# kabachuha/sd-webui-text2video

Hardware: NVIDIA H100
Metric: denoised frames/sec (UNet+VAE) ModelScope 24fx256^2 50-step (higher is better)
Workload: dtype f16 (fp32 accumulate / norms / softmax)

## Files before the change

### include/t2v_b200.h

```cpp
#ifndef T2V_B200_H
#define T2V_B200_H

#include <stddef.h>
#include <stdint.h>

#ifdef __cplusplus
extern "C" {
#endif

int t2v_init(int device);
const char* t2v_last_error(void);
int t2v_num_sms(void);
const char* t2v_version(void);

typedef struct t2v_unet t2v_unet;

typedef struct {
    int in_dim, dim, context_dim, out_dim;
    int dim_mult[8];
    int n_mult;
    int num_heads;
    int head_dim;
    int num_res_blocks;
    float attn_scales[8];
    int n_attn_scales;
    int arch;
    int temporal_length;
} t2v_unet_config;

int t2v_unet_create(const t2v_unet_config* cfg, t2v_unet** out);
void t2v_unet_destroy(t2v_unet* u);
int t2v_unet_set_param(t2v_unet* u, const char* name, const void* data, int dtype, int ndim, const int64_t* shape,
                       void* stream);
int t2v_unet_missing_params(t2v_unet* u, char* name_out, size_t name_cap);
int t2v_unet_param_info(t2v_unet* u, int index, char* name_out, size_t name_cap, int64_t* shape_out, int* ndim_out);
int t2v_unet_forward(t2v_unet* u, const void* x, int x_is_f32, const float* t, const void* ctx, void* out,
                     int out_is_f32, int B, int F, int h, int w, int L, void* stream);
int t2v_unet_forward_ctx(t2v_unet* u, const void* x, int x_is_f32, const float* t, const void* ctx, int ctx_B, void* out,
                         int out_is_f32, int B, int F, int h, int w, int L, void* stream);
int t2v_unet_forward_adapter(t2v_unet* u, const void* x, int x_is_f32, const float* t, const void* ctx,
                             const void* const* feats, int n_feats, int feats_B, void* out, int out_is_f32, int B, int F, int h,
                             int w, int L, void* stream);
double t2v_unet_flops(t2v_unet* u, int B, int F, int h, int w, int L);
int t2v_unet_plan_bytes(t2v_unet* u, int B, int F, int h, int w, int L, size_t* arena);
int t2v_unet_plan_info(t2v_unet* u, int B, int ctx_B, int F, int h, int w, int L, size_t* arena, double* flops, int* cached);
int t2v_unet_num_launches(t2v_unet* u);
int t2v_unet_profile(t2v_unet* u, int B, int F, int h, int w, int L, void* stream, double* out13);
long long t2v_unet_read_tap(t2v_unet* u, const char* name, void* dst, long long cap_elems, void* stream);
int t2v_unet_enable_taps(t2v_unet* u, int on);
int t2v_unet_tap_info(t2v_unet* u, const char* name, long long* rows, int* C, int* h, int* w);

int t2v_unet_lora_merge(t2v_unet* u, const char* weight_name, const void* lora_A, const void* lora_B, int rank, float alpha,
                        int temporal_mean, void* stream);
int t2v_unet_lora_clear(t2v_unet* u, void* stream);
int t2v_unet_lora_merged(t2v_unet* u);

int t2v_unet_lora_apply(t2v_unet* u, const char* weight_name, const void* up, const void* down, int dtype, int rank, float alpha,
                        void* stream);
int t2v_unet_lora_restore(t2v_unet* u, const char* weight_name, void* stream);

typedef struct {
    unsigned char comm_handle[64];
    unsigned char slab_handle[64];
    int rank, nranks;
    int n_exchanges, n_groupnorms;
    long long dst_offset[192];
} t2v_shard_export;
int t2v_unet_shard_setup(t2v_unet* u, int rank, int nranks);
int t2v_unet_shard_prepare(t2v_unet* u, int B, int F, int h, int w, int L, void* stream, t2v_shard_export* out);
int t2v_unet_shard_connect(t2v_unet* u, int B, int F, int h, int w, int L, const t2v_shard_export* all, void* stream);
int t2v_unet_shard_connected(t2v_unet* u, int B, int F, int h, int w, int L);
int t2v_unet_shard_barrier(t2v_unet* u, void* stream);
int t2v_unet_shard_info(t2v_unet* u, int F, int* frame_begin, int* frame_end, int* n_exchanges);

typedef struct t2v_vae t2v_vae;
typedef struct {
    int ch;
    int ch_mult[8];
    int n_mult;
    int num_res_blocks;
    int z_channels;
    int out_ch;
    int embed_dim;
} t2v_vae_config;
int t2v_vae_create(const t2v_vae_config* cfg, t2v_vae** out);
void t2v_vae_destroy(t2v_vae* v);
int t2v_vae_set_param(t2v_vae* v, const char* name, const void* data, int dtype, int ndim, const int64_t* shape,
                      void* stream);
int t2v_vae_missing_params(t2v_vae* v, char* name_out, size_t name_cap);
int t2v_vae_param_info(t2v_vae* v, int index, char* name_out, size_t name_cap, int64_t* shape_out, int* ndim_out);
int t2v_vae_decode(t2v_vae* v, const void* z, int z_is_f32, float z_scale, void* out, int out_mode, int B, int F, int h,
                   int w, void* stream);
int t2v_vae_encode(t2v_vae* v, const void* x, int x_is_f32, void* moments_out, int N, int H, int W, void* stream);
double t2v_vae_flops(t2v_vae* v, int nframes, int h, int w);
int t2v_vae_plan_bytes(t2v_vae* v, int direction, int frames, int h, int w, size_t* arena, size_t* gn_workspace);
int t2v_vae_plan_chunks(t2v_vae* v, int direction, int frames, int h, int w, size_t budget, int* chunk_frames, int* n_chunks);
int t2v_vae_set_memory_budget(t2v_vae* v, size_t bytes);
size_t t2v_vae_get_memory_budget(t2v_vae* v);
int t2v_vae_last_chunking(t2v_vae* v, int direction, int* chunk_frames, int* n_chunks);
int t2v_vae_cached_plans(t2v_vae* v, int direction, size_t* slab_bytes);
int t2v_vae_lora_apply(t2v_vae* v, const char* weight_name, const void* up, const void* down, int dtype, int rank, float alpha,
                       void* stream);
int t2v_vae_lora_restore(t2v_vae* v, const char* weight_name, void* stream);
int t2v_vae_lora_clear(t2v_vae* v, void* stream);
int t2v_vae_lora_merged(t2v_vae* v);

typedef struct t2v_clip t2v_clip;
typedef struct {
    int width;
    int heads;
    int layers_run;
    int context;
    int vocab;
    int arch;
} t2v_clip_config;
int t2v_clip_create(const t2v_clip_config* cfg, t2v_clip** out);
void t2v_clip_destroy(t2v_clip* m);
int t2v_clip_set_param(t2v_clip* m, const char* name, const void* data, int dtype, int ndim, const int64_t* shape, void* stream);
int t2v_clip_param_info(t2v_clip* m, int index, char* name_out, size_t name_cap, int64_t* shape_out, int* ndim_out);
int t2v_clip_encode(t2v_clip* m, const int* tokens, void* out, int out_is_f32, int B, void* stream);
int t2v_clip_lora_apply(t2v_clip* m, const char* weight_name, const void* up, const void* down, int dtype, int rank, float alpha,
                        void* stream);
int t2v_clip_lora_restore(t2v_clip* m, const char* weight_name, void* stream);
int t2v_clip_lora_clear(t2v_clip* m, void* stream);
int t2v_clip_lora_merged(t2v_clip* m);

typedef struct t2v_adapter t2v_adapter;
typedef struct {
    int cin;
    int channels[4];
    int n_levels;
    int nums_rb;
    int ksize;
    int sk;
    int use_conv;
} t2v_adapter_config;
int t2v_adapter_create(const t2v_adapter_config* cfg, t2v_adapter** out);
void t2v_adapter_destroy(t2v_adapter* a);
int t2v_adapter_set_param(t2v_adapter* a, const char* name, const void* data, int dtype, int ndim, const int64_t* shape,
                          void* stream);
int t2v_adapter_missing_params(t2v_adapter* a, char* name_out, size_t name_cap);
int t2v_adapter_param_info(t2v_adapter* a, int index, char* name_out, size_t name_cap, int64_t* shape_out, int* ndim_out);
int t2v_adapter_encode(t2v_adapter* a, const void* cond, int cond_is_f32, void* const* feats_out, int N, int H, int W,
                       void* stream);
int t2v_adapter_lora_apply(t2v_adapter* a, const char* weight_name, const void* up, const void* down, int dtype, int rank,
                           float alpha, void* stream);
int t2v_adapter_lora_restore(t2v_adapter* a, const char* weight_name, void* stream);
int t2v_adapter_lora_clear(t2v_adapter* a, void* stream);
int t2v_adapter_lora_merged(t2v_adapter* a);

int t2v_ddim_step(const float* x, const void* eps_c, const void* eps_u, int eps_is_f32, float* x_out, long long n,
                  long long chan_stride,
                  int C, int guided_channels, float g, int mode, float a0, float a1, float a2, float a3, float a4,
                  const float* noise, int cfg_fp16, void* stream);
int t2v_cfg_x0(const float* x, const void* eps_c, const void* eps_u, int eps_is_f32, float* x0, long long n, float g,
               float alpha, float sigma, int cfg_fp16, void* stream);
int t2v_lincomb(float* out, const float* const* src, const float* coef, int n_src, long long n, void* stream);

int t2v_latent_blend(const float* image_latents, int image_frames, const double* noise, const double* weights, double* out,
                     double* mask_out, int BC, int F, long long hw, void* stream);

int t2v_q_sample_blend(const float* x0, const long long* x0_strides, const float* noise, const long long* noise_strides,
                       const float* a, const float* s, const float* mask, const long long* mask_strides, const float* img,
                       float* out, const int* shape, void* stream);

int t2v_frames_resize(const void* src, int n, int H0, int W0, void* out, int H, int W, int out_fp16, void* tmp,
                      long long tmp_bytes, void* stream);
int t2v_resize_coeffs(int in_size, int out_size, int* ksize, int* bounds, int* coeffs);

int t2v_op_gemm(const void* a, long long lda, int K, int nd, const int* dims, int ntaps, const int* tap_off,
                const void* w_packed, int n_alloc, int N, int b_batch_dim, int flags, void* out, long long ldo,
                const void* bias, int bias_rows, long long bias_stride, const void* residual, long long ldr,
                float alpha, int force_bn, int force_cg, void* stream);
int t2v_op_gemm_splitk(const void* a, long long lda, int K, int nd, const int* dims, int ntaps, const int* tap_off,
                       const void* w_packed, int n_alloc, int N, int b_batch_dim, int flags, void* out, long long ldo,
                       const void* bias, int bias_rows, long long bias_stride, const void* residual, long long ldr,
                       float alpha, int splits, float* scratch, long long scratch_elems, int* splits_used, int force_bn,
                       int force_cg, void* stream);
int t2v_op_ln_linear(const void* x, long long ldx, long long rows, int K, const void* w, const void* bias, const void* gamma,
                     const void* beta, int N, int flags, void* w_folded, float* colsum, float* bias32, float* rowstat,
                     const void* residual, long long ldr, void* out, long long ldo, int force_bn, int force_cg, void* stream);
int t2v_op_pack_conv_weight(const void* src, int src_is_f32, void* dst, int Cout, int Cin, int taps, int n_alloc,
                            int k_alloc, void* stream);
int t2v_op_pack_geglu_weight(const void* w, const void* b, int src_is_f32, void* wdst, void* bdst, int H, int K, int bn,
                             void* stream);
int t2v_op_groupnorm(const void* x, long long ldx, void* y, long long ldy, long long rows, int C, int rows_per_inst,
                     const void* gamma, const void* beta, float eps, int silu, int phase, float* stats, void* stream);
int t2v_op_layernorm(const void* x, long long ldx, void* y, long long ldy, long long rows, int C, const void* gamma,
                     const void* beta, float eps, void* stream);
int t2v_op_attention(const void* q, const void* k, const void* v, void* o, long long q_bs, long long q_ss,
                     long long k_bs, long long k_ss, long long v_bs, long long v_ss, long long o_bs, long long o_ss,
                     int batch, int heads, int sq, int skv, int kv_batch_div, float scale, void* stream);
int t2v_op_attention_hd(const void* q, const void* k, const void* v, void* o, long long q_bs, long long q_ss,
                        long long k_bs, long long k_ss, long long v_bs, long long v_ss, long long o_bs, long long o_ss,
                        int batch, int heads, int head_dim, int sq, int skv, int kv_batch_div, float scale, int b_inner,
                        long long q_bsi, long long k_bsi, long long v_bsi, long long o_bsi, void* stream);
int t2v_op_attention_relpos(const void* q, const void* k, const void* v, void* o, const void* table_k, const void* table_v,
                            long long n_seq, long long seq_inner, long long bs_outer, long long bs_inner, long long ss,
                            long long o_bs_outer, long long o_bs_inner, long long o_ss, int heads, int head_dim, int T,
                            int max_rel, float scale, void* stream);
int t2v_op_clip_attention(const void* qkv, void* o, int B, int L, int W, int heads, void* stream);
int t2v_op_upsample2x(const void* x, void* y, int nframes, int h, int w, int C, void* stream);
int t2v_op_im2col_s2(const void* x, void* col, int nframes, int h, int w, int C, void* stream);
int t2v_op_time_sinusoid(const float* t, void* out, int B, int dim, void* stream);
int t2v_op_small_linear(const void* x, long long ldx, const void* W, const void* bias, const void* addend, void* y,
                        long long ldy, int B, int N, int K, int silu_in, void* stream);

#ifdef __cplusplus
}
#endif
#endif
```

### sd-webui-text2video_b200/csrc/api.cu

```cuda
#include "../../include/t2v_b200.h"
#include "common.cuh"
#include "gemm_tc.cuh"
#include "kernels.cuh"

#include <cstdarg>
#include <cstdio>
#include <cstring>

namespace t2v {

static char g_err[512] = "";
static int g_device = -1;
static int g_num_sms = 132;
static void* g_gn_ws = nullptr;
static size_t g_gn_ws_bytes = 0;

void set_error(const char* fmt, ...) {
    va_list ap;
    va_start(ap, fmt);
    vsnprintf(g_err, sizeof(g_err), fmt, ap);
    va_end(ap);
}
int num_sms() { return g_num_sms; }
void clear_pending_error(const char* where) {
    const cudaError_t e = cudaGetLastError();
    if (e != cudaSuccess)
        fprintf(stderr, "[t2v_b200] %s: clearing a pending CUDA error left by an earlier call: %s (%s)\n", where, cudaGetErrorString(e),
                cudaGetErrorName(e));
}
int launch_status(const char* what) {
    const cudaError_t e = cudaGetLastError();
    if (e == cudaSuccess) return 0;
    set_error("%s: %s (%s)", what, cudaGetErrorString(e), cudaGetErrorName(e));
    return -2;
}

static void* gn_scratch(size_t bytes) {
    if (bytes > g_gn_ws_bytes) {
        if (g_gn_ws) cudaFree(g_gn_ws);
        g_gn_ws = nullptr;
        if (cudaMalloc(&g_gn_ws, bytes) != cudaSuccess) return nullptr;
        cudaMemset(g_gn_ws, 0, bytes);
        g_gn_ws_bytes = bytes;
    }
    return g_gn_ws;
}

}

using namespace t2v;

extern "C" {

int t2v_init(int device) {
    if (cudaSetDevice(device) != cudaSuccess) {
        set_error("cudaSetDevice(%d) failed: %s", device, cudaGetErrorString(cudaGetLastError()));
        return -1;
    }
    cudaDeviceProp prop;
    if (cudaGetDeviceProperties(&prop, device) != cudaSuccess) {
        set_error("cudaGetDeviceProperties failed");
        return -1;
    }
    if (prop.major != 9 || prop.minor != 0) {
        set_error("t2v_b200 is built for sm_90a only; device %d is sm_%d%d", device, prop.major, prop.minor);
        return -2;
    }
    g_device = device;
    g_num_sms = prop.multiProcessorCount;
    if (gemm_init() != 0) {
        set_error("gemm_init failed (driver entry point / smem attribute)");
        return -3;
    }
    return 0;
}
const char* t2v_last_error(void) { return g_err; }
int t2v_num_sms(void) { return g_num_sms; }
const char* t2v_version(void) { return "t2v_b200 0.2 (sm_90a; wgmma+TMA implicit GEMM)"; }

}

static GemmProblem op_problem(const void* a, long long lda, int K, int nd, const int* dims, int ntaps, const int* tap_off,
                              const void* w_packed, int n_alloc, int N, int b_batch_dim, int flags, void* out, long long ldo,
                              const void* bias, int bias_rows, long long bias_stride, const void* residual, long long ldr,
                              float alpha, int force_bn, int force_cg) {
    GemmProblem p;
    memset(&p, 0, sizeof(p));
    p.a = reinterpret_cast<const __half*>(a);
    p.lda = lda;
    p.K = K;
    p.nd = nd;
    for (int d = 0; d < nd; ++d) p.dim[d] = dims[d];
    p.ntaps = ntaps;
    for (int t = 0; t < ntaps; ++t)
        for (int d = 0; d < nd; ++d) p.tap_off[t][d] = tap_off ? tap_off[t * nd + d] : 0;
    p.b = reinterpret_cast<const __half*>(w_packed);
    p.n_alloc = n_alloc;
    p.N = N;
    p.b_batch_dim = b_batch_dim;
    p.flags = flags & ~(GEMM_DBG_FORCE_BS | GEMM_DBG_NO_BS | GEMM_DBG_SLAB_OUT);
    p.force_bs = (flags & GEMM_DBG_FORCE_BS) ? 1 : ((flags & GEMM_DBG_NO_BS) ? -1 : 0);
    p.slab_out = (flags & GEMM_DBG_SLAB_OUT) ? 1 : 0;
    p.out = out;
    p.ldo = ldo;
    p.bias = reinterpret_cast<const __half*>(bias);
    p.bias_rows = bias_rows;
    p.bias_stride = bias_stride;
    p.residual = reinterpret_cast<const __half*>(residual);
    p.ldr = ldr;
    p.alpha = alpha;
    p.force_bn = force_bn;
    p.force_cg = force_cg;
    return p;
}

static int plan_op(const GemmProblem& p, GemmPlan* plan, const char* what) {
    const int rc = gemm_plan(p, plan, g_num_sms);
    if (rc != 0) set_error("%s: gemm_plan failed (%d)", what, rc);
    return rc;
}

static int launch_op(const GemmPlan& plan, const char* what, cudaStream_t stream) {
    const int rc = gemm_launch(plan, stream);
    if (rc != 0) set_error("%s: gemm_launch failed: %s", what, cudaGetErrorString(cudaGetLastError()));
    return rc;
}

extern "C" {

int t2v_op_gemm(const void* a, long long lda, int K, int nd, const int* dims, int ntaps, const int* tap_off,
                const void* w_packed, int n_alloc, int N, int b_batch_dim, int flags, void* out, long long ldo,
                const void* bias, int bias_rows, long long bias_stride, const void* residual, long long ldr,
                float alpha, int force_bn, int force_cg, void* stream) {
    const GemmProblem p = op_problem(a, lda, K, nd, dims, ntaps, tap_off, w_packed, n_alloc, N, b_batch_dim, flags, out, ldo, bias,
                                     bias_rows, bias_stride, residual, ldr, alpha, force_bn, force_cg);
    GemmPlan plan;
    const int rc = plan_op(p, &plan, "op_gemm");
    return rc != 0 ? rc : launch_op(plan, "op_gemm", reinterpret_cast<cudaStream_t>(stream));
}

int t2v_op_gemm_splitk(const void* a, long long lda, int K, int nd, const int* dims, int ntaps, const int* tap_off,
                       const void* w_packed, int n_alloc, int N, int b_batch_dim, int flags, void* out, long long ldo,
                       const void* bias, int bias_rows, long long bias_stride, const void* residual, long long ldr,
                       float alpha, int splits, float* scratch, long long scratch_elems, int* splits_used, int force_bn,
                       int force_cg, void* stream) {
    const GemmProblem p = op_problem(a, lda, K, nd, dims, ntaps, tap_off, w_packed, n_alloc, N, b_batch_dim, flags, out, ldo, bias,
                                     bias_rows, bias_stride, residual, ldr, alpha, force_bn, force_cg);
    if (const char* why = gemm_splitk_unsupported(p)) {
        set_error("op_gemm_splitk: split-K does not take this problem: %s", why);
        return -1;
    }
    if (splits < 1 || scratch == nullptr || splits_used == nullptr) {
        set_error("op_gemm_splitk: needs splits >= 1, a scratch buffer and a place for the split count");
        return -1;
    }
    const int S = gemm_split_count(p, splits);
    const long long need = gemm_splitk_scratch_elems(p, S);
    if (scratch_elems < need) {
        set_error("op_gemm_splitk: %d splits need %lld fp32 scratch elements, the buffer holds %lld", S, need, scratch_elems);
        return -1;
    }
    GemmPlan plan;
    int rc = plan_op(gemm_splitk_partials(p, S, scratch), &plan, "op_gemm_splitk");
    if (rc != 0) return rc;
    *splits_used = S;
    const cudaStream_t s = reinterpret_cast<cudaStream_t>(stream);
    rc = launch_op(plan, "op_gemm_splitk", s);
    if (rc != 0) return rc;
    rc = gemm_splitk_reduce(p, S, scratch, s);
    if (rc != 0) set_error("op_gemm_splitk: splitk_reduce failed (%d)", rc);
    return rc;
}

int t2v_op_ln_linear(const void* x, long long ldx, long long rows, int K, const void* w, const void* bias, const void* gamma,
                     const void* beta, int N, int flags, void* w_folded, float* colsum, float* bias32, float* rowstat,
                     const void* residual, long long ldr, void* out, long long ldo, int force_bn, int force_cg, void* stream) {
    if (!x || !w || !gamma || !beta || !w_folded || !colsum || !bias32 || !rowstat || !out) {
        set_error("op_ln_linear: x, w, gamma, beta, out and the four intermediate buffers are required");
        return -1;
    }
    if ((flags & ~GEMM_GEGLU) != 0) {
        set_error("op_ln_linear: flags must be 0 or GEMM_GEGLU (%d)", flags);
        return -1;
    }
    if (K % 8 != 0 || K > 2048 || rows < 1 || rows >= (1LL << 31) || N < 1) {
        set_error("op_ln_linear: LayerNorm rows need K %% 8 == 0 and K <= 2048, 1 <= rows < 2^31 (K %d rows %lld N %d)", K, rows, N);
        return -1;
    }
    GemmProblem p;
    memset(&p, 0, sizeof(p));
    p.a = reinterpret_cast<const __half*>(x);
    p.lda = ldx;
    p.K = K;
    p.nd = 1;
    p.dim[0] = static_cast<int>(rows);
    p.ntaps = 1;
    p.b = reinterpret_cast<const __half*>(w_folded);
    p.n_alloc = N;
    p.N = N;
    p.b_batch_dim = -1;
    p.flags = flags | GEMM_LN;
    p.out = out;
    p.ldo = ldo;
    p.residual = reinterpret_cast<const __half*>(residual);
    p.ldr = ldr;
    p.alpha = 1.0f;
    p.force_bn = force_bn;
    p.force_cg = force_cg;
    p.rowstat = reinterpret_cast<const float2*>(rowstat);
    p.colsum = colsum;
    p.bias32 = bias32;
    GemmPlan plan;
    int rc = plan_op(p, &plan, "op_ln_linear");
    if (rc != 0) return rc;
    const cudaStream_t s = reinterpret_cast<cudaStream_t>(stream);
    rc = fold_ln_into_linear(reinterpret_cast<const __half*>(w), reinterpret_cast<const __half*>(bias),
                             reinterpret_cast<const __half*>(gamma), reinterpret_cast<const __half*>(beta),
                             reinterpret_cast<__half*>(w_folded), colsum, bias32, N, K, s);
    if (rc == 0) rc = layernorm_rowstats(p.a, ldx, rows, K, 1e-5f, reinterpret_cast<float2*>(rowstat), s);
    if (rc != 0) {
        set_error("op_ln_linear: fold / row statistics launch failed (%d)", rc);
        return rc;
    }
    return launch_op(plan, "op_ln_linear", s);
}

int t2v_latent_blend(const float* image_latents, int image_frames, const double* noise, const double* weights, double* out,
                     double* mask_out, int BC, int F, long long hw, void* stream) {
    if ((image_frames != 1 && image_frames != F) || BC < 1 || F < 1 || hw < 1) {
        set_error("latent_blend: image_frames must be 1 or F");
        return -1;
    }
    return latent_blend(image_latents, image_frames, noise, weights, out, mask_out, BC, F, hw, reinterpret_cast<cudaStream_t>(stream));
}

int t2v_q_sample_blend(const float* x0, const long long* x0_strides, const float* noise, const long long* noise_strides,
                       const float* a, const float* s, const float* mask, const long long* mask_strides, const float* img,
                       float* out, const int* shape, void* stream) {
    if (!x0 || !x0_strides || !noise || !noise_strides || !a || !s || !out || !shape) {
        set_error("q_sample_blend: x0, noise, a, s, out, their strides and the shape are required");
        return -1;
    }
    if ((mask == nullptr) != (img == nullptr) || (mask && !mask_strides)) {
        set_error("q_sample_blend: mask and img go together (both null for q_sample), and a mask needs strides");
        return -1;
    }
    QSampleBlendParams p;
    memset(&p, 0, sizeof(p));
    p.x0 = x0;
    p.noise = noise;
    p.a = a;
    p.s = s;
    p.mask = mask;
    p.img = img;
    p.out = out;
    for (int d = 0; d < 5; ++d) {
        if (shape[d] < 1) {
            set_error("q_sample_blend: shape[%d] = %d, every dimension must be >= 1", d, shape[d]);
            return -1;
        }
        if (x0_strides[d] < 0 || noise_strides[d] < 0 || (mask && mask_strides[d] < 0)) {
            set_error("q_sample_blend: negative stride in dimension %d", d);
            return -1;
        }
        p.shape[d] = shape[d];
        p.x0_stride[d] = x0_strides[d];
        p.noise_stride[d] = noise_strides[d];
        p.mask_stride[d] = mask ? mask_strides[d] : 0;
    }
    return q_sample_blend(p, reinterpret_cast<cudaStream_t>(stream));
}

int t2v_resize_coeffs(int in_size, int out_size, int* ksize, int* bounds, int* coeffs) {
    if (ksize == nullptr || resize_table(in_size, out_size, ksize, bounds, coeffs) != 0) {
        set_error("resize_coeffs: sizes must lie in [1, %d] (in %d, out %d) and ksize must not be null", kResizeMaxSize, in_size,
                  out_size);
        return -1;
    }
    return 0;
}

int t2v_frames_resize(const void* src, int n, int H0, int W0, void* out, int H, int W, int out_fp16, void* tmp,
                      long long tmp_bytes, void* stream) {
    const int M = kResizeMaxSize;
    if (n < 1 || H0 < 1 || W0 < 1 || H < 1 || W < 1 || H0 > M || W0 > M || H > M || W > M) {
        set_error("frames_resize: n must be >= 1 and every size in [1, %d] (n %d, %dx%d -> %dx%d)", M, n, W0, H0, W, H);
        return -1;
    }
    if (src == nullptr || out == nullptr) {
        set_error("frames_resize: src and out are required");
        return -1;
    }
    const size_t esize = out_fp16 ? sizeof(__half) : sizeof(float);
    if (reinterpret_cast<uintptr_t>(out) % esize != 0) {
        set_error("frames_resize: out must be aligned to its element size (%zu bytes)", esize);
        return -1;
    }
    const long long need = W != W0 ? static_cast<long long>(n) * H0 * W * 3 : 0;
    if (W != W0 && (tmp == nullptr || tmp_bytes < need)) {
        set_error("frames_resize: resizing %d to %d columns needs a uint8 buffer of %lld bytes, got %lld", W0, W, need,
                  tmp ? tmp_bytes : 0LL);
        return -1;
    }
    clear_pending_error("frames_resize");
    return frames_resize(static_cast<const uint8_t*>(src), n, H0, W0, out, H, W, out_fp16, static_cast<uint8_t*>(tmp),
                         reinterpret_cast<cudaStream_t>(stream));
}

int t2v_op_pack_conv_weight(const void* src, int src_is_f32, void* dst, int Cout, int Cin, int taps, int n_alloc,
                            int k_alloc, void* stream) {
    return pack_conv_weight(src, src_is_f32, reinterpret_cast<__half*>(dst), Cout, Cin, taps, n_alloc, k_alloc,
                            reinterpret_cast<cudaStream_t>(stream));
}
int t2v_op_pack_geglu_weight(const void* w, const void* b, int src_is_f32, void* wdst, void* bdst, int H, int K, int bn,
                             void* stream) {
    return pack_geglu_weight(w, b, src_is_f32, reinterpret_cast<__half*>(wdst), reinterpret_cast<__half*>(bdst), H, K, bn,
                             reinterpret_cast<cudaStream_t>(stream));
}
int t2v_op_groupnorm(const void* x, long long ldx, void* y, long long ldy, long long rows, int C, int rows_per_inst,
                     const void* gamma, const void* beta, float eps, int silu, int phase, float* stats, void* stream) {
    const __half* xh = reinterpret_cast<const __half*>(x);
    __half* yh = reinterpret_cast<__half*>(y);
    const __half* gh = reinterpret_cast<const __half*>(gamma);
    const __half* bh = reinterpret_cast<const __half*>(beta);
    if (phase < 0 || phase > 2 || (phase != 0 && stats == nullptr)) {
        set_error("op_groupnorm: phase %d must be 0, 1 or 2, and phases 1 and 2 need a stats buffer", phase);
        return -1;
    }
    if (groupnorm_check(xh, ldx, yh, ldy, rows, C, rows_per_inst, gh, bh) != 0) return -1;
    const int n_inst = static_cast<int>(rows / rows_per_inst);
    void* ws = gn_scratch(gn_workspace_bytes(rows_per_inst, n_inst, g_num_sms));
    if (!ws) {
        set_error("groupnorm workspace allocation failed");
        return -5;
    }
    const cudaStream_t s = reinterpret_cast<cudaStream_t>(stream);
    const size_t stats_bytes = static_cast<size_t>(n_inst) * 32 * sizeof(float2);
    if (phase == 2 && cudaMemcpyAsync(gn_workspace_stats(ws), stats, stats_bytes, cudaMemcpyDeviceToDevice, s) != cudaSuccess)
        return launch_status("op_groupnorm: statistics copy");
    const int rc = groupnorm_silu(xh, ldx, yh, ldy, rows, C, rows_per_inst, gh, bh, eps, silu, ws, g_num_sms, s, phase);
    if (rc != 0 || phase != 1) return rc;
    if (cudaMemcpyAsync(stats, gn_workspace_stats(ws), stats_bytes, cudaMemcpyDeviceToDevice, s) != cudaSuccess)
        return launch_status("op_groupnorm: statistics copy");
    return 0;
}
int t2v_op_layernorm(const void* x, long long ldx, void* y, long long ldy, long long rows, int C, const void* gamma,
                     const void* beta, float eps, void* stream) {
    return layernorm(reinterpret_cast<const __half*>(x), ldx, reinterpret_cast<__half*>(y), ldy, rows, C,
                     reinterpret_cast<const __half*>(gamma), reinterpret_cast<const __half*>(beta), eps,
                     reinterpret_cast<cudaStream_t>(stream));
}
int t2v_op_attention(const void* q, const void* k, const void* v, void* o, long long q_bs, long long q_ss,
                     long long k_bs, long long k_ss, long long v_bs, long long v_ss, long long o_bs, long long o_ss,
                     int batch, int heads, int sq, int skv, int kv_batch_div, float scale, void* stream) {
    AttnParams p;
    p.q = reinterpret_cast<const __half*>(q);
    p.k = reinterpret_cast<const __half*>(k);
    p.v = reinterpret_cast<const __half*>(v);
    p.o = reinterpret_cast<__half*>(o);
    p.q_bs = q_bs; p.q_ss = q_ss; p.k_bs = k_bs; p.k_ss = k_ss; p.v_bs = v_bs; p.v_ss = v_ss; p.o_bs = o_bs; p.o_ss = o_ss;
    p.batch = batch; p.heads = heads; p.sq = sq; p.skv = skv; p.head_dim = 64; p.kv_batch_div = kv_batch_div;
    p.scale = scale; p.b_inner = 1; p.q_bsi = p.k_bsi = p.v_bsi = p.o_bsi = 0;
    return attention(p, reinterpret_cast<cudaStream_t>(stream));
}
int t2v_op_attention_hd(const void* q, const void* k, const void* v, void* o, long long q_bs, long long q_ss,
                        long long k_bs, long long k_ss, long long v_bs, long long v_ss, long long o_bs, long long o_ss,
                        int batch, int heads, int head_dim, int sq, int skv, int kv_batch_div, float scale, int b_inner,
                        long long q_bsi, long long k_bsi, long long v_bsi, long long o_bsi, void* stream) {
    AttnParams p;
    memset(&p, 0, sizeof(p));
    p.q = reinterpret_cast<const __half*>(q);
    p.k = reinterpret_cast<const __half*>(k);
    p.v = reinterpret_cast<const __half*>(v);
    p.o = reinterpret_cast<__half*>(o);
    p.q_bs = q_bs; p.q_ss = q_ss; p.k_bs = k_bs; p.k_ss = k_ss; p.v_bs = v_bs; p.v_ss = v_ss; p.o_bs = o_bs; p.o_ss = o_ss;
    p.batch = batch; p.heads = heads; p.sq = sq; p.skv = skv; p.head_dim = head_dim; p.kv_batch_div = kv_batch_div;
    p.scale = scale; p.b_inner = b_inner;
    p.q_bsi = q_bsi; p.k_bsi = k_bsi; p.v_bsi = v_bsi; p.o_bsi = o_bsi;
    return attention(p, reinterpret_cast<cudaStream_t>(stream));
}
int t2v_op_attention_relpos(const void* q, const void* k, const void* v, void* o, const void* table_k, const void* table_v,
                            long long n_seq, long long seq_inner, long long bs_outer, long long bs_inner, long long ss,
                            long long o_bs_outer, long long o_bs_inner, long long o_ss, int heads, int head_dim, int T,
                            int max_rel, float scale, void* stream) {
    RelposParams p;
    memset(&p, 0, sizeof(p));
    p.q = reinterpret_cast<const __half*>(q);
    p.k = reinterpret_cast<const __half*>(k);
    p.v = reinterpret_cast<const __half*>(v);
    p.o = reinterpret_cast<__half*>(o);
    p.table_k = reinterpret_cast<const __half*>(table_k);
    p.table_v = reinterpret_cast<const __half*>(table_v);
    p.n_seq = n_seq; p.seq_inner = seq_inner; p.bs_outer = bs_outer; p.bs_inner = bs_inner; p.ss = ss;
    p.o_bs_outer = o_bs_outer; p.o_bs_inner = o_bs_inner; p.o_ss = o_ss;
    p.heads = heads; p.head_dim = head_dim; p.T = T; p.max_rel = max_rel; p.scale = scale;
    return attention_relpos(p, reinterpret_cast<cudaStream_t>(stream));
}
int t2v_op_upsample2x(const void* x, void* y, int nframes, int h, int w, int C, void* stream) {
    return upsample2x(reinterpret_cast<const __half*>(x), reinterpret_cast<__half*>(y), nframes, h, w, C,
                      reinterpret_cast<cudaStream_t>(stream));
}
int t2v_op_im2col_s2(const void* x, void* col, int nframes, int h, int w, int C, void* stream) {
    return im2col_s2(reinterpret_cast<const __half*>(x), reinterpret_cast<__half*>(col), nframes, h, w, C,
                     reinterpret_cast<cudaStream_t>(stream));
}
int t2v_op_time_sinusoid(const float* t, void* out, int B, int dim, void* stream) {
    return time_sinusoid(t, reinterpret_cast<__half*>(out), B, dim, reinterpret_cast<cudaStream_t>(stream));
}
int t2v_op_small_linear(const void* x, long long ldx, const void* W, const void* bias, const void* addend, void* y,
                        long long ldy, int B, int N, int K, int silu_in, void* stream) {
    return small_linear(reinterpret_cast<const __half*>(x), ldx, reinterpret_cast<const __half*>(W),
                        reinterpret_cast<const __half*>(bias), reinterpret_cast<const __half*>(addend),
                        reinterpret_cast<__half*>(y), ldy, B, N, K, silu_in, reinterpret_cast<cudaStream_t>(stream));
}
int t2v_ddim_step(const float* x, const void* eps_c, const void* eps_u, int eps_is_f32, float* x_out, long long n, long long chan_stride,
                  int C, int guided_channels, float g, int mode, float a0, float a1, float a2, float a3, float a4,
                  const float* noise, int cfg_fp16, void* stream) {
    DdimStepParams p;
    p.x = x; p.eps_c = eps_c; p.eps_u = eps_u; p.eps_is_f32 = eps_is_f32;
    p.x_out = x_out; p.n = n; p.chan_stride = chan_stride; p.C = C; p.guided_channels = guided_channels; p.g = g;
    p.mode = mode; p.a0 = a0; p.a1 = a1; p.a2 = a2; p.a3 = a3; p.a4 = a4; p.noise = noise; p.cfg_fp16 = cfg_fp16;
    return ddim_step(p, reinterpret_cast<cudaStream_t>(stream));
}
int t2v_cfg_x0(const float* x, const void* eps_c, const void* eps_u, int eps_is_f32, float* x0, long long n, float g, float alpha,
               float sigma, int cfg_fp16, void* stream) {
    return cfg_x0(x, eps_c, eps_u, eps_is_f32, x0, n, g, alpha, sigma,
                  cfg_fp16, reinterpret_cast<cudaStream_t>(stream));
}
int t2v_lincomb(float* out, const float* const* src, const float* coef, int n_src, long long n, void* stream) {
    return lincomb(out, src, coef, n_src, n, reinterpret_cast<cudaStream_t>(stream));
}

}
```

### sd-webui-text2video_b200/csrc/gemm_tc.cu

```cuda
#include "common.cuh"
#include "gemm_tc.cuh"
#include "kernels.cuh"
#include "ptx.cuh"

#include <algorithm>
#include <cstdio>
#include <cstdlib>
#include <cstring>

namespace t2v {

namespace {

constexpr int kThreads = 384;
constexpr int kRegsProducer = 40;
constexpr int kRegsConsumer = 232;
constexpr int kABytes = GEMM_BLOCK_M * GEMM_BLOCK_K * 2;
constexpr int kSmemPerBlock = 227 * 1024;
constexpr int kSmemBudget = 216 * 1024;
constexpr int kMaxStages = 8;
constexpr int kEpiRowBytes = 128;
constexpr int kSlabBytes = 8 * 8 * kEpiRowBytes;
constexpr int kRowTabBytes = 8 * 16 * 4;

__host__ __device__ constexpr int out_chunk_cols(int outw) { return outw >= 32 ? 32 : 16; }
__host__ __device__ constexpr int out_chunks(int outw) { return (outw + out_chunk_cols(outw) - 1) / out_chunk_cols(outw); }

template <int BN, bool SLAB = false>
struct Cfg {
    static constexpr int kBBytes = BN * GEMM_BLOCK_K * 2;
    static constexpr int kStageBytes = kABytes + kBBytes;
    static constexpr int kColBytes = BN * 8;
    static constexpr int kTailBytes = 1024  + 256  + kRowTabBytes + kColBytes;
    static constexpr int kOutBytes = SLAB ? kSlabBytes : std::max(kSlabBytes, out_chunks(BN) * GEMM_BLOCK_M * out_chunk_cols(BN) * 2);
    static constexpr int kStages = std::min(kMaxStages, (kSmemPerBlock - kTailBytes - kOutBytes) / kStageBytes);
    static constexpr int kSmemBytes = kStages * kStageBytes + kOutBytes + kTailBytes;
    static constexpr int kBsSmemBytes = kSmemBudget + kSlabBytes + kTailBytes;
    static_assert(kSmemBytes <= kSmemPerBlock, "shared memory per block");
};
static_assert(Cfg<256>::kStages == 3 && Cfg<224>::kStages == 3 && Cfg<192>::kStages == 4 && Cfg<160>::kStages == 5 &&
                  Cfg<128>::kStages == 6 && Cfg<64>::kStages == 8 && Cfg<16>::kStages == 8,
              "ring depths next to the output tile");
static_assert(Cfg<256, true>::kStages == 4 && Cfg<224, true>::kStages == 4, "ring depths without the output tile");

__device__ __forceinline__ float gelu_erf(float x) {
    const float z = fabsf(x) * 0.70710678118654752440f;
    float t;
    asm("rcp.approx.ftz.f32 %0, %1;" : "=f"(t) : "f"(fmaf(0.3275911f, z, 1.0f)));
    float p = fmaf(t, 0.5f * 1.061405429f, 0.5f * -1.453152027f);
    p = fmaf(p, t, 0.5f * 1.421413741f);
    p = fmaf(p, t, 0.5f * -0.284496736f);
    p = fmaf(p, t, 0.5f * 0.254829592f);
    const float q = p * t * ex2_approx(z * z * -1.4426950408889634f);
    return x * (x < 0.f ? q : 1.0f - q);
}

__device__ __forceinline__ uint32_t stg_off(int r, int b, int segs) {
    const int L = r * segs + (b >> 4);
    return static_cast<uint32_t>(((L ^ ((L >> 3) & 7)) << 4) | (b & 15));
}

template <int BN, bool GEGLU>
__device__ __forceinline__ void epilogue_affine(const GemmDesc& g, float (&acc)[BN / 2], const uint8_t* cols, const int* rowg,
                                                const float2 (&rs)[2], int tn, int lane) {
    const int quad = lane & 3, fr = lane >> 2;
    if (!GEGLU && g.bias != nullptr && g.bias_rows > 0 && (g.flags & GEMM_LN) == 0) {
        const int col0 = tn * BN + 2 * quad;
        const int nrem = g.N - col0;
        const __half* brow[2];
#pragma unroll
        for (int h = 0; h < 2; ++h) {
            const int fg = rowg[fr + 8 * h];
            brow[h] = g.bias + (fg >= 0 ? (fg / g.bias_rows) * g.bias_stride : 0) + col0;
        }
#pragma unroll
        for (int j = 0; j < BN / 8; ++j) {
#pragma unroll
            for (int e = 0; e < 2; ++e) {
                if (8 * j + e >= nrem) continue;
                acc[4 * j + e] = fmaf(acc[4 * j + e], g.alpha, __half2float(__ldg(brow[0] + 8 * j + e)));
                acc[4 * j + 2 + e] = fmaf(acc[4 * j + 2 + e], g.alpha, __half2float(__ldg(brow[1] + 8 * j + e)));
            }
        }
        return;
    }
    const bool ln = (g.flags & GEMM_LN) != 0;
#pragma unroll
    for (int j = 0; j < BN / 8; ++j) {
        const int c = 8 * j + 2 * quad;
        if (ln) {
            const float4 p = *reinterpret_cast<const float4*>(cols + 8 * c);
            acc[4 * j] = fmaf(rs[0].y, fmaf(-rs[0].x, p.x, acc[4 * j]), p.y);
            acc[4 * j + 2] = fmaf(rs[1].y, fmaf(-rs[1].x, p.x, acc[4 * j + 2]), p.y);
            acc[4 * j + 1] = fmaf(rs[0].y, fmaf(-rs[0].x, p.z, acc[4 * j + 1]), p.w);
            acc[4 * j + 3] = fmaf(rs[1].y, fmaf(-rs[1].x, p.z, acc[4 * j + 3]), p.w);
        } else {
            const float2 b = __half22float2(*reinterpret_cast<const __half2*>(cols + 2 * c));
            acc[4 * j] = fmaf(acc[4 * j], g.alpha, b.x);
            acc[4 * j + 2] = fmaf(acc[4 * j + 2], g.alpha, b.x);
            acc[4 * j + 1] = fmaf(acc[4 * j + 1], g.alpha, b.y);
            acc[4 * j + 3] = fmaf(acc[4 * j + 3], g.alpha, b.y);
        }
    }
}

template <int BN>
struct ResQ {
    static constexpr int kCW = kEpiRowBytes / 2;
    static constexpr int kUnits = 2 * ((BN + kCW - 1) / kCW);
    static constexpr int kDepth = BN <= 192 ? kUnits : 4;
    static __device__ __forceinline__ int segs(int c) { return (min(kCW, BN - c * kCW) * 2) / 16; }
    static __device__ __forceinline__ void load(const GemmDesc& g, const int* rowg, int tn, int u, int lane, uint4 (&rb)[2]) {
        const int c = u >> 1, h = u & 1, sg = segs(c);
        const bool vec_res = (g.ldr & 7) == 0 && (reinterpret_cast<uintptr_t>(g.residual) & 15) == 0;
#pragma unroll
        for (int p = 0; p < 2; ++p) {
            const int idx = lane + 32 * p;
            rb[p] = make_uint4(0u, 0u, 0u, 0u);
            if (idx >= 8 * sg) continue;
            const int gr = rowg[8 * h + idx / sg];
            const int col = tn * BN + c * kCW + 8 * (idx % sg);
            if (gr < 0) continue;
            const __half* src = g.residual + gr * g.ldr + col;
            if (vec_res && col + 8 <= g.N) {
                rb[p] = __ldg(reinterpret_cast<const uint4*>(src));
            } else {
                uint32_t w[4];
#pragma unroll
                for (int e = 0; e < 4; ++e) {
                    const __half2 v = __halves2half2(col + 2 * e < g.N ? src[2 * e] : __ushort_as_half(0),
                                                     col + 2 * e + 1 < g.N ? src[2 * e + 1] : __ushort_as_half(0));
                    w[e] = *reinterpret_cast<const uint32_t*>(&v);
                }
                rb[p] = make_uint4(w[0], w[1], w[2], w[3]);
            }
        }
    }
};

template <int BN, bool GEGLU, bool F32>
__device__ __forceinline__ void epilogue_warp(const GemmDesc& g, float (&acc)[BN / 2], uint4 (&rq)[ResQ<BN>::kDepth][2],
                                              uint8_t* stg, const int* rowg, int tn, int sp, int lane) {
    static_assert(!(GEGLU && F32), "GEGLU stores fp16");
    constexpr bool RES = !GEGLU && !F32;
    constexpr int ES = F32 ? 4 : 2;
    constexpr int EPS = 16 / ES;
    constexpr int OUTW = GEGLU ? BN / 2 : BN;
    constexpr int CW = kEpiRowBytes / ES;
    constexpr int NCH = (OUTW + CW - 1) / CW;
    constexpr int NU = 2 * NCH;
    constexpr int QD = ResQ<BN>::kDepth;
    const int quad = lane & 3, fr = lane >> 2;
    const int nvalid = GEGLU ? g.N / 2 : g.N;
    const int ocol0 = tn * OUTW;
    const bool has_res = RES && g.residual != nullptr;
    const bool vec_out = (g.ldo % EPS) == 0 && (reinterpret_cast<uintptr_t>(g.out) & 15) == 0 && (!F32 || (g.split_stride % EPS) == 0);

    auto segs_of = [](int c) { return (min(CW, OUTW - c * CW) * ES) / 16; };
#pragma unroll
    for (int u = 0; u < NU; ++u) {
        const int c = u >> 1, h = u & 1, segs = segs_of(c);
        if (RES && has_res) {
#pragma unroll
            for (int p = 0; p < 2; ++p) {
                const int idx = lane + 32 * p;
                if (idx < 8 * segs) *reinterpret_cast<uint4*>(stg + stg_off(idx / segs, 16 * (idx % segs), segs)) = rq[u % QD][p];
            }
            if (u + QD < NU) ResQ<BN>::load(g, rowg, tn, u + QD, lane, rq[u % QD]);
            __syncwarp();
        }
#pragma unroll
        for (int jj = 0; jj < CW / 8; ++jj) {
            if (jj >= segs * EPS / 8) break;
            const int j = c * (CW / 8) + jj;
            uint8_t* sp_ = stg + stg_off(fr, (8 * jj + 2 * quad) * ES, segs);
            float v0 = acc[4 * j + 2 * h], v1 = acc[4 * j + 2 * h + 1];
            if constexpr (GEGLU) {
                const __half2 xh = __floats2half2_rn(v0, v1);
                const float2 gf = __half22float2(__floats2half2_rn(acc[BN / 4 + 4 * j + 2 * h], acc[BN / 4 + 4 * j + 2 * h + 1]));
                const __half2 ge = __floats2half2_rn(gelu_erf(gf.x), gelu_erf(gf.y));
                *reinterpret_cast<__half2*>(sp_) = __hmul2(xh, ge);
            } else if constexpr (F32) {
                *reinterpret_cast<float2*>(sp_) = make_float2(v0, v1);
            } else {
                if (has_res) {
                    const float2 f = __half22float2(*reinterpret_cast<const __half2*>(sp_));
                    v0 += f.x;
                    v1 += f.y;
                }
                *reinterpret_cast<__half2*>(sp_) = __floats2half2_rn(v0, v1);
            }
        }
        __syncwarp();
#pragma unroll
        for (int p = 0; p < 2; ++p) {
            const int idx = lane + 32 * p;
            if (idx >= 8 * segs) continue;
            const int gr = rowg[8 * h + idx / segs];
            if (gr < 0) continue;
            const int col = ocol0 + c * CW + EPS * (idx % segs);
            const uint4 val = *reinterpret_cast<const uint4*>(stg + stg_off(idx / segs, 16 * (idx % segs), segs));
            uint8_t* dst = static_cast<uint8_t*>(g.out) + ((F32 ? sp * g.split_stride : 0) + gr * g.ldo + col) * ES;
            if (vec_out && col + EPS <= nvalid) {
                *reinterpret_cast<uint4*>(dst) = val;
            } else {
                const uint32_t w[4] = {val.x, val.y, val.z, val.w};
#pragma unroll
                for (int e = 0; e < EPS; ++e)
                    if (col + e < nvalid) {
                        if constexpr (F32) reinterpret_cast<uint32_t*>(dst)[e] = w[e];
                        else reinterpret_cast<uint16_t*>(dst)[e] = static_cast<uint16_t>(w[e >> 1] >> (16 * (e & 1)));
                    }
            }
        }
        __syncwarp();
    }
}

__device__ __forceinline__ void tile_origin(const GemmDesc& g, int tmi, int (&org)[GEMM_MAX_RDIMS]) {
#pragma unroll
    for (int d = 0; d < GEMM_MAX_RDIMS; ++d) org[d] = 0;
    if (g.nd == 1) {
        org[0] = tmi * g.box[0];
        return;
    }
    int tm = tmi;
#pragma unroll
    for (int d = 0; d < GEMM_MAX_RDIMS; ++d) {
        if (d < g.nd) {
            const int td = g.tdim[d];
            const int qd = tm / td;
            org[d] = (tm - qd * td) * g.box[d];
            tm = qd;
        }
    }
}

__device__ __forceinline__ void tma_store_box(const CUtensorMap* map, const void* src, int nd, int c0, const int (&org)[GEMM_MAX_RDIMS]) {
    if (nd == 1) tma_store_2d(map, src, c0, org[0]);
    else if (nd == 2) tma_store_3d(map, src, c0, org[0], org[1]);
    else if (nd == 3) tma_store_4d(map, src, c0, org[0], org[1], org[2]);
    else tma_store_5d(map, src, c0, org[0], org[1], org[2], org[3]);
}
__device__ __forceinline__ void tma_load_box(void* dst, const CUtensorMap* map, uint64_t* bar, int nd, int c0,
                                             const int (&org)[GEMM_MAX_RDIMS]) {
    if (nd == 1) tma_load_2d(dst, map, bar, c0, org[0]);
    else if (nd == 2) tma_load_3d(dst, map, bar, c0, org[0], org[1]);
    else if (nd == 3) tma_load_4d(dst, map, bar, c0, org[0], org[1], org[2]);
    else tma_load_5d(dst, map, bar, c0, org[0], org[1], org[2], org[3]);
}

template <int OCW>
__device__ __forceinline__ int out_unit_swizzle(int r) { return ((r * OCW * 2) >> 7) & (OCW / 8 - 1); }

template <int BN, bool GEGLU>
__device__ __forceinline__ int live_out_chunks(const GemmDesc& g, int tn) {
    constexpr int OUTW = GEGLU ? BN / 2 : BN;
    constexpr int OCW = out_chunk_cols(OUTW);
    return min(out_chunks(OUTW), ((GEGLU ? g.N / 2 : g.N) - tn * OUTW + OCW - 1) / OCW);
}

template <int BN, bool GEGLU>
__device__ __forceinline__ void epilogue_tile(const GemmDesc& g, const float (&acc)[BN / 2], uint8_t* tile, uint64_t* tilefree,
                                              uint32_t tphase, uint64_t* tilefull, int r0, int lane) {
    constexpr int OUTW = GEGLU ? BN / 2 : BN;
    constexpr int OCW = out_chunk_cols(OUTW);
    const int quad = lane & 3, fr = lane >> 2;
    const bool has_res = !GEGLU && g.residual != nullptr;
    const uint32_t row = smem_u32(tile) + static_cast<uint32_t>((r0 + fr) * (OCW * 2) + 4 * quad);
    const int sw = out_unit_swizzle<OCW>(r0 + fr);
    mbar_wait(tilefree, tphase);
#pragma unroll
    for (int j = 0; j < OUTW / 8; ++j) {
#pragma unroll
        for (int h = 0; h < 2; ++h) {
            const uint32_t p = row + (j / (OCW / 8)) * (GEMM_BLOCK_M * OCW * 2) + 8 * h * (OCW * 2) + (((j % (OCW / 8)) ^ sw) << 4);
            float v0 = acc[4 * j + 2 * h], v1 = acc[4 * j + 2 * h + 1];
            __half2 v;
            if constexpr (GEGLU) {
                const __half2 xh = __floats2half2_rn(v0, v1);
                const float2 gf = __half22float2(__floats2half2_rn(acc[BN / 4 + 4 * j + 2 * h], acc[BN / 4 + 4 * j + 2 * h + 1]));
                v = __hmul2(xh, __floats2half2_rn(gelu_erf(gf.x), gelu_erf(gf.y)));
            } else {
                if (has_res) {
                    const uint32_t rw = ld_shared_u32(p);
                    const float2 f = __half22float2(*reinterpret_cast<const __half2*>(&rw));
                    v0 += f.x;
                    v1 += f.y;
                }
                v = __floats2half2_rn(v0, v1);
            }
            st_shared_u32(p, *reinterpret_cast<const uint32_t*>(&v));
        }
    }
    fence_proxy_async_smem();
    __syncwarp();
    if (lane == 0) mbar_arrive(tilefull);
}

template <int BN, bool GEGLU, int CG, bool BS = false, bool SLAB = false>
__global__ void __launch_bounds__(kThreads, 1) gemm_tc_kernel(const __grid_constant__ GemmDesc g) {
    using Cf = Cfg<BN, SLAB>;
    static_assert(!BS || CG == 1, "B-stationary tiles are single-CTA");
    static_assert(!BS || Cf::kBsSmemBytes <= kSmemPerBlock, "shared memory per block");
    constexpr int kBarStages = BS ? kMaxStages : Cf::kStages;
    const uint32_t rank = CG == 2 ? cluster_ctarank() : 0u;
    extern __shared__ uint8_t smem_raw[];
    const uint32_t raw = smem_u32(smem_raw);
    uint8_t* smem = smem_raw + (((raw + 1023u) & ~1023u) - raw);
    uint8_t* const epi = smem + (BS ? kSmemBudget : Cf::kStages * Cf::kStageBytes);
    uint64_t* bars = reinterpret_cast<uint64_t*>(epi + (BS ? kSlabBytes : Cf::kOutBytes));
    uint64_t* full = bars;
    uint64_t* empty = bars + kBarStages;
    uint64_t* bfull = empty + kBarStages;
    uint64_t* colfull = bfull + 1;
    uint64_t* colempty = bfull + 2;
    uint64_t* tilefree = bfull + 3;
    uint64_t* tilefull = bfull + 4;
    int* const rowtab = reinterpret_cast<int*>(reinterpret_cast<uint8_t*>(bars) + 256);
    uint8_t* const cols = reinterpret_cast<uint8_t*>(rowtab) + kRowTabBytes;
    const bool tma_out = !BS && !SLAB && g.tma_out != 0;
    const int nst = BS ? g.bs_stages : Cf::kStages;
    uint8_t* const sB_res = smem;
    uint8_t* const sA_ring = smem + (BS ? g.ntaps * g.k_chunks * Cf::kBBytes : 0);

    const int wg = threadIdx.x >> 7;

    if (threadIdx.x == 0) {
        tma_prefetch_desc(&g.map_a);
        tma_prefetch_desc(&g.map_b);
        if (tma_out) {
            tma_prefetch_desc(&g.map_o);
            if (g.residual != nullptr) tma_prefetch_desc(&g.map_r);
        }
        for (int i = 0; i < kBarStages; ++i) {
            mbar_init(&full[i], 1);
            mbar_init(&empty[i], 2 * CG);
        }
        if constexpr (BS) mbar_init(bfull, 1);
        mbar_init(colfull, 1);
        mbar_init(colempty, 8);
        mbar_init(tilefree, 1);
        mbar_init(tilefull, 8);
        fence_barrier_init();
    }
    if constexpr (CG == 2) cluster_sync_all();
    else __syncthreads();

    const int pairs_m = (g.tiles_m + CG - 1) / CG;
    const int nsplit = g.splits > 1 ? g.splits : 1;
    const int total_pairs = pairs_m * g.tiles_n * nsplit;
    const int k_total = g.ntaps * g.k_chunks;
    const int k_per = g.splits > 1 ? g.k_per_split : k_total;
    const int bs_tn = BS ? static_cast<int>(blockIdx.x) % g.tiles_n : 0;
    const int first_pair = BS ? static_cast<int>(blockIdx.x) / g.tiles_n : static_cast<int>(blockIdx.x) / CG;
    const int pair_stride = BS ? (static_cast<int>(gridDim.x) - bs_tn + g.tiles_n - 1) / g.tiles_n : static_cast<int>(gridDim.x) / CG;
    const int total_items = BS ? g.tiles_m : total_pairs;
    const bool col_operands = (g.flags & GEMM_LN) != 0 || g.bias == nullptr || g.bias_rows == 0;

    if (wg == 0) {
        setmaxnreg_dec<kRegsProducer>();
        if (threadIdx.x < 32 && elect_one()) {
            int stage = 0;
            uint32_t phase = 0;
            if constexpr (BS) {
                if (first_pair < total_items) {
                    mbar_expect_tx(bfull, static_cast<uint32_t>(k_total * Cf::kBBytes));
                    const int kch0 = g.k_chunks;
                    for (int it = 0, tap = 0, kc = 0; it < k_total; ++it) {
                        tma_load_3d(sB_res + it * Cf::kBBytes, &g.map_b, bfull, kc * GEMM_BLOCK_K, bs_tn * BN, tap);
                        if (++kc == kch0) {
                            kc = 0;
                            ++tap;
                        }
                    }
                }
            }
            const int kch = g.k_chunks, nd = g.nd, a_tx = g.a_tx_bytes, tiles_n_ = g.tiles_n, tiles_m_ = g.tiles_m;
            const int bdim = g.b_batch_dim;
            for (int wi = first_pair; wi < total_items; wi += pair_stride) {
                int sp = 0, pt = wi;
                if (!BS && nsplit > 1) {
                    sp = wi % nsplit;
                    pt = wi / nsplit;
                }
                const int it0 = sp * k_per, it1 = min(k_total, it0 + k_per);
                int tn = bs_tn, tmi = wi;
                if constexpr (!BS) {
                    const int pm = pt / tiles_n_;
                    tn = pt - pm * tiles_n_;
                    tmi = pm * CG + static_cast<int>(rank);
                }
                int org[GEMM_MAX_RDIMS];
                tile_origin(g, tmi, org);
                if (tmi >= tiles_m_) org[0] = g.dim[0];
                const int bbatch = bdim < 0 ? 0 : (bdim == 0 ? org[0] : (bdim == 1 ? org[1] : (bdim == 2 ? org[2] : org[3])));
                int tap = 0, kc = it0;
                if (it0 >= kch) {
                    tap = it0 / kch;
                    kc = it0 - tap * kch;
                }
                int c1 = org[0] + g.tap_off[tap][0], c2 = org[1] + g.tap_off[tap][1];
                int c3 = org[2] + g.tap_off[tap][2], c4 = org[3] + g.tap_off[tap][3];
                for (int it = it0; it < it1; ++it) {
                    mbar_wait(&empty[stage], phase ^ 1u);
                    uint8_t* sa = BS ? sA_ring + stage * kABytes : smem + stage * Cf::kStageBytes;
                    uint8_t* sb = sa + kABytes;
                    const int k0 = kc * GEMM_BLOCK_K;
                    mbar_expect_tx(&full[stage], static_cast<uint32_t>(a_tx + (BS ? 0 : Cf::kBBytes)));
                    if (nd == 1) tma_load_2d(sa, &g.map_a, &full[stage], k0, c1);
                    else if (nd == 2) tma_load_3d(sa, &g.map_a, &full[stage], k0, c1, c2);
                    else if (nd == 3) tma_load_4d(sa, &g.map_a, &full[stage], k0, c1, c2, c3);
                    else tma_load_5d(sa, &g.map_a, &full[stage], k0, c1, c2, c3, c4);
                    if constexpr (CG == 2) {
                        constexpr int kHalf = BN / 2;
                        tma_load_3d_mc(sb + rank * (kHalf * GEMM_BLOCK_K * 2), &g.map_b, &full[stage], k0,
                                       tn * BN + static_cast<int>(rank) * kHalf, tap + bbatch, static_cast<uint16_t>(3));
                    } else if constexpr (!BS) {
                        tma_load_3d(sb, &g.map_b, &full[stage], k0, tn * BN, tap + bbatch);
                    }
                    if (++kc == kch) {
                        kc = 0;
                        ++tap;
                        if (it + 1 < it1) {
                            c1 = org[0] + g.tap_off[tap][0];
                            c2 = org[1] + g.tap_off[tap][1];
                            c3 = org[2] + g.tap_off[tap][2];
                            c4 = org[3] + g.tap_off[tap][3];
                        }
                    }
                    if (++stage == nst) {
                        stage = 0;
                        phase ^= 1u;
                    }
                }
            }
        } else if (threadIdx.x >= 32 && threadIdx.x < 64 && col_operands) {
            const int lane = threadIdx.x & 31;
            const bool ln = (g.flags & GEMM_LN) != 0;
            uint32_t cphase = 0;
            for (int wi = first_pair; wi < total_items; wi += pair_stride) {
                const int col0 = (BS ? bs_tn : (wi / nsplit) % g.tiles_n) * BN;
                mbar_wait(colempty, cphase ^ 1u);
#pragma unroll
                for (int c = lane; c < BN; c += 32) {
                    const int col = col0 + c;
                    if (ln) {
                        reinterpret_cast<float2*>(cols)[c] =
                            col < g.N ? make_float2(__ldg(g.colsum + col), __ldg(g.bias32 + col)) : make_float2(0.f, 0.f);
                    } else {
                        reinterpret_cast<__half*>(cols)[c] = g.bias != nullptr && col < g.N ? __ldg(g.bias + col) : __ushort_as_half(0);
                    }
                }
                __syncwarp();
                if (lane == 0) mbar_arrive(colfull);
                cphase ^= 1u;
            }
        } else if (threadIdx.x >= 64 && threadIdx.x < 96 && tma_out) {
            if (elect_one()) {
                constexpr int OUTW = GEGLU ? BN / 2 : BN;
                constexpr int OCW = out_chunk_cols(OUTW);
                constexpr int kChunkBytes = GEMM_BLOCK_M * OCW * 2;
                const bool has_res = !GEGLU && g.residual != nullptr;
                const uint32_t box_bytes = static_cast<uint32_t>(g.a_tx_bytes / GEMM_BLOCK_K * OCW);
                uint32_t fphase = 0;
                for (int wi = first_pair; wi < total_items; wi += pair_stride) {
                    const int pt = wi / nsplit;
                    const int tn = pt % g.tiles_n;
                    const int tmi = (pt / g.tiles_n) * CG + static_cast<int>(rank);
                    const int nch = tmi < g.tiles_m ? live_out_chunks<BN, GEGLU>(g, tn) : 0;
                    int org[GEMM_MAX_RDIMS];
                    tile_origin(g, tmi, org);
                    if (has_res && nch > 0) {
                        mbar_expect_tx(tilefree, nch * box_bytes);
                        for (int c = 0; c < nch; ++c)
                            tma_load_box(epi + c * kChunkBytes, &g.map_r, tilefree, g.nd, tn * OUTW + c * OCW, org);
                    } else {
                        mbar_arrive(tilefree);
                    }
                    mbar_wait(tilefull, fphase);
                    fphase ^= 1u;
                    for (int c = 0; c < nch; ++c) tma_store_box(&g.map_o, epi + c * kChunkBytes, g.nd, tn * OUTW + c * OCW, org);
                    bulk_commit_group();
                    bulk_wait_group_read_0();
                }
                bulk_wait_group_0();
            }
        }
        __syncwarp();
    } else {
        setmaxnreg_inc<kRegsConsumer>();
        const int cw = wg - 1;
        const int lt = threadIdx.x & 127;
        const int wr = lt >> 5, lane = lt & 31;
        int stage = 0;
        uint32_t phase = 0;
        if constexpr (BS) {
            if (first_pair < total_items) mbar_wait(bfull, 0u);
        }
        const bool out_f32 = (g.flags & GEMM_OUT_F32) != 0;
        const bool ln = (g.flags & GEMM_LN) != 0;
        uint8_t* const stg = epi + (cw * 4 + wr) * (8 * kEpiRowBytes);
        int* const rowg = rowtab + (cw * 4 + wr) * 16;
        uint32_t cphase = 0, tphase = 0;
        float acc[BN / 2];
        uint4 rq[ResQ<BN>::kDepth][2];
        for (int wi = first_pair; wi < total_items; wi += pair_stride) {
            const int sp = BS ? 0 : wi % nsplit;
            const int pt = wi / nsplit;
            const int tn = BS ? bs_tn : pt % g.tiles_n;
            const int tmi = BS ? wi : (pt / g.tiles_n) * CG + static_cast<int>(rank);
            const int it0s = BS ? 0 : sp * k_per;
            const int k_iters = min(g.ntaps * g.k_chunks, it0s + k_per) - it0s;

            if (lane < 16) {
                const int r = cw * 64 + wr * 16 + lane;
                int grow = -1;
                if (tmi < g.tiles_m) {
                    if (g.nd == 1) {
                        const int o = tmi * g.box[0];
                        if (r < g.box[0] && o + r < g.dim[0]) grow = o + r;
                    } else {
                        int tm = tmi, rr = r;
                        long long mul = 1, gr = 0;
                        bool valid = true;
#pragma unroll
                        for (int d = 0; d < GEMM_MAX_RDIMS; ++d) {
                            const int td = g.tdim[d];
                            const int c = (tm % td) * g.box[d] + rr % g.box[d];
                            tm /= td;
                            rr /= g.box[d];
                            valid = valid && (c < g.dim[d]);
                            gr += mul * c;
                            mul *= g.dim[d];
                        }
                        if (valid && rr == 0) grow = static_cast<int>(gr);
                    }
                }
                rowg[lane] = grow;
            }
            __syncwarp();
            float2 rs[2];
#pragma unroll
            for (int h = 0; h < 2; ++h) {
                const int fg = rowg[(lane >> 2) + 8 * h];
                rs[h] = ln && fg >= 0 ? __ldg(g.rowstat + fg) : make_float2(0.f, 1.f);
            }

            int prev = -1;
#pragma unroll
            for (int i = 0; i < BN / 2; ++i) reg_fence(acc[i]);
            for (int it = 0; it < k_iters; ++it) {
                mbar_wait(&full[stage], phase);
                const uint32_t sa = smem_u32(BS ? sA_ring + stage * kABytes : smem + stage * Cf::kStageBytes) + cw * (64 * 128);
                const uint32_t sb = BS ? smem_u32(sB_res + it * Cf::kBBytes) : smem_u32(smem + stage * Cf::kStageBytes) + kABytes;
                const uint64_t da = wgmma_desc_sw128(sa);
                const uint64_t db = wgmma_desc_sw128(sb);
                wgmma_fence();
#pragma unroll
                for (int k = 0; k < GEMM_BLOCK_K / 16; ++k)
                    wgmma_ss<BN>(acc, da + static_cast<uint64_t>(k * 2), db + static_cast<uint64_t>(k * 2), (it | k) != 0 ? 1u : 0u);
                wgmma_commit();
                wgmma_wait<1>();
                if (prev >= 0 && lt == 0) {
                    mbar_arrive(&empty[prev]);
                    if constexpr (CG == 2) mbar_arrive_cluster(&empty[prev], rank ^ 1u);
                }
                prev = stage;
                if (++stage == nst) {
                    stage = 0;
                    phase ^= 1u;
                }
            }
            if constexpr (!GEGLU) {
                if (!tma_out && g.residual != nullptr) {
#pragma unroll
                    for (int u = 0; u < ResQ<BN>::kDepth; ++u) ResQ<BN>::load(g, rowg, tn, u, lane, rq[u]);
                }
            }
            wgmma_wait<0>();
#pragma unroll
            for (int i = 0; i < BN / 2; ++i) reg_fence(acc[i]);
            if (prev >= 0 && lt == 0) {
                mbar_arrive(&empty[prev]);
                if constexpr (CG == 2) mbar_arrive_cluster(&empty[prev], rank ^ 1u);
            }

            uint32_t ring = static_cast<uint32_t>(stage) | (phase << 16);
            asm volatile("" : "+r"(ring));
            if (col_operands) mbar_wait(colfull, cphase);
            epilogue_affine<BN, GEGLU>(g, acc, cols, rowg, rs, tn, lane);
            if (col_operands) {
                __syncwarp();
                if (lane == 0) mbar_arrive(colempty);
                cphase ^= 1u;
            }
            if (tma_out) {
                epilogue_tile<BN, GEGLU>(g, acc, epi, tilefree, tphase, tilefull, cw * 64 + wr * 16, lane);
                tphase ^= 1u;
            } else if constexpr (GEGLU) {
                epilogue_warp<BN, true, false>(g, acc, rq, stg, rowg, tn, sp, lane);
            } else if (out_f32) {
                epilogue_warp<BN, false, true>(g, acc, rq, stg, rowg, tn, sp, lane);
            } else {
                epilogue_warp<BN, false, false>(g, acc, rq, stg, rowg, tn, sp, lane);
            }
            asm volatile("" : "+r"(ring));
            stage = static_cast<int>(ring & 0xffffu);
            phase = ring >> 16;
        }
    }
    if constexpr (CG == 2) cluster_sync_all();
}

typedef CUresult (*EncodeTiledFn)(CUtensorMap*, CUtensorMapDataType, cuuint32_t, void*, const cuuint64_t*,
                                  const cuuint64_t*, const cuuint32_t*, const cuuint32_t*, CUtensorMapInterleave,
                                  CUtensorMapSwizzle, CUtensorMapL2promotion, CUtensorMapFloatOOBfill);
EncodeTiledFn g_encode = nullptr;
bool g_inited = false;

int encode_map(CUtensorMap* m, const void* base, int rank, const cuuint64_t* dims, const cuuint64_t* strides_bytes,
               const cuuint32_t* box, CUtensorMapSwizzle swizzle = CU_TENSOR_MAP_SWIZZLE_128B) {
    cuuint32_t estr[5] = {1, 1, 1, 1, 1};
    CUresult r = g_encode(m, CU_TENSOR_MAP_DATA_TYPE_FLOAT16, static_cast<cuuint32_t>(rank), const_cast<void*>(base),
                          dims, strides_bytes, box, estr, CU_TENSOR_MAP_INTERLEAVE_NONE, swizzle,
                          CU_TENSOR_MAP_L2_PROMOTION_L2_256B, CU_TENSOR_MAP_FLOAT_OOB_FILL_NONE);
    if (r != CUDA_SUCCESS) {
        fprintf(stderr, "[t2v] cuTensorMapEncodeTiled failed: %d (rank %d, dims %llu %llu %llu %llu %llu)\n",
                static_cast<int>(r), rank, (unsigned long long)dims[0], (unsigned long long)(rank > 1 ? dims[1] : 0),
                (unsigned long long)(rank > 2 ? dims[2] : 0), (unsigned long long)(rank > 3 ? dims[3] : 0),
                (unsigned long long)(rank > 4 ? dims[4] : 0));
        return -1;
    }
    return 0;
}

struct Variant {
    int bn, geglu, cg, smem;
    const void* fn;
    int bs, slab;
};
template <int BN, bool G, int CG>
Variant variant() {
    return Variant{BN, G ? 1 : 0, CG, Cfg<BN>::kSmemBytes, reinterpret_cast<const void*>(&gemm_tc_kernel<BN, G, CG>), 0, 0};
}
template <int BN, bool G>
Variant variant_bs() {
    return Variant{BN, G ? 1 : 0, 1, Cfg<BN>::kBsSmemBytes, reinterpret_cast<const void*>(&gemm_tc_kernel<BN, G, 1, true>), 1, 0};
}
template <int BN>
Variant variant_slab() {
    return Variant{BN, 0, 1, Cfg<BN, true>::kSmemBytes, reinterpret_cast<const void*>(&gemm_tc_kernel<BN, false, 1, false, true>), 0, 1};
}
const Variant* variants(int* n) {
    static const Variant v[] = {
        variant<16, false, 1>(),  variant<64, false, 1>(),  variant<128, false, 1>(), variant<160, false, 1>(),
        variant<192, false, 1>(), variant<224, false, 1>(),
        variant<256, false, 1>(), variant<64, true, 1>(),   variant<128, true, 1>(),  variant<256, true, 1>(),
        variant<64, false, 2>(),  variant<128, false, 2>(), variant<160, false, 2>(), variant<256, false, 2>(),
        variant<64, true, 2>(),   variant<128, true, 2>(),  variant<256, true, 2>(),
        variant_bs<160, false>(), variant_bs<128, false>(), variant_bs<128, true>(), variant_bs<64, false>(),
        variant_slab<224>(),      variant_slab<256>(),
    };
    *n = static_cast<int>(sizeof(v) / sizeof(v[0]));
    return v;
}
const Variant* find_variant(int bn, bool geglu, int cg, int bs, int slab) {
    int n;
    const Variant* v = variants(&n);
    for (int i = 0; i < n; ++i)
        if (v[i].bn == bn && v[i].geglu == (geglu ? 1 : 0) && v[i].cg == cg && v[i].bs == bs && v[i].slab == slab) return &v[i];
    return nullptr;
}

}

int gemm_init() {
    if (g_inited) return 0;
    void* fn = nullptr;
    cudaDriverEntryPointQueryResult qres;
    if (cudaGetDriverEntryPoint("cuTensorMapEncodeTiled", &fn, cudaEnableDefault, &qres) != cudaSuccess ||
        fn == nullptr) {
        fprintf(stderr, "[t2v] cuTensorMapEncodeTiled entry point not found\n");
        return -1;
    }
    g_encode = reinterpret_cast<EncodeTiledFn>(fn);
    int nv = 0;
    const Variant* vs = variants(&nv);
    bool attr_fail = false;
    for (int i = 0; i < nv; ++i)
        if (cudaFuncSetAttribute(vs[i].fn, cudaFuncAttributeMaxDynamicSharedMemorySize, vs[i].smem) != cudaSuccess) attr_fail = true;
    if (attr_fail) {
        fprintf(stderr, "[t2v] cudaFuncSetAttribute(max dynamic smem) failed: %s\n",
                cudaGetErrorString(cudaGetLastError()));
        return -1;
    }
    g_inited = true;
    return 0;
}

int tma_encode_f16(CUtensorMap* m, const void* base, int rank, const unsigned long long* dims,
                   const unsigned long long* strides_bytes, const unsigned* box) {
    if (gemm_init() != 0) return -1;
    cuuint64_t d[5], st[5];
    cuuint32_t bx[5];
    for (int i = 0; i < rank; ++i) {
        d[i] = dims[i];
        bx[i] = box[i];
        if (i + 1 < rank) st[i] = strides_bytes[i];
    }
    return encode_map(m, base, rank, d, st, bx);
}

static int gemm_bs_bn(long long tiles_m, int N, int K, int ntaps, int num_sms, int force_bn, bool any_k, int* stages_out) {
    static const bool bs_off = getenv("T2V_NO_BSTAT") != nullptr;
    static const int bs_kmax = getenv("T2V_BSTAT_KMAX") ? atoi(getenv("T2V_BSTAT_KMAX")) : 0;
    const int kt = ntaps * ((K + GEMM_BLOCK_K - 1) / GEMM_BLOCK_K);
    if (bs_off || N <= 16 || (kt > bs_kmax && !any_k)) return 0;
    const int cands[3] = {160, 128, 64};
    for (int i = 0; i < 3; ++i) {
        const int c = cands[i];
        if (force_bn != 0 && force_bn != c) continue;
        const int tn = (N + c - 1) / c;
        if (static_cast<double>(N) / (static_cast<double>(tn) * c) < 0.9) continue;
        const long long b_bytes = static_cast<long long>(kt) * c * GEMM_BLOCK_K * 2;
        if (b_bytes > kSmemBudget - 4 * kABytes || tn > num_sms) continue;
        const int stages = static_cast<int>(std::min<long long>(8, (kSmemBudget - b_bytes) / kABytes));
        const int group = num_sms / tn;
        if (tiles_m < 3LL * group) continue;
        if (stages_out) *stages_out = stages;
        return c;
    }
    return 0;
}

int gemm_plan(const GemmProblem& p, GemmPlan* plan, int num_sms) {
    if (gemm_init() != 0) return -1;
    if (p.nd < 1 || p.nd > GEMM_MAX_RDIMS || p.ntaps < 1 || p.ntaps > GEMM_MAX_TAPS) return -2;
    if ((p.lda & 7) != 0 || (p.K & 7) != 0 || (reinterpret_cast<uintptr_t>(p.a) & 15) != 0 ||
        (reinterpret_cast<uintptr_t>(p.b) & 15) != 0) {
        fprintf(stderr, "[t2v] gemm_plan: operands must be 16-byte aligned (lda %lld K %d)\n", p.lda, p.K);
        return -3;
    }
    GemmDesc& g = plan->desc;
    memset(&g, 0, sizeof(g));
    g.nd = p.nd;
    long long rows = 1;
    int remaining = GEMM_BLOCK_M;
    int boxrows = 1;
    for (int d = 0; d < GEMM_MAX_RDIMS; ++d) {
        const int ext = d < p.nd ? p.dim[d] : 1;
        g.dim[d] = ext;
        int b = std::min(ext, remaining);
        if (b < 1) b = 1;
        g.box[d] = b;
        g.tdim[d] = (ext + b - 1) / b;
        remaining = b >= ext ? remaining / b : 1;
        boxrows *= b;
        rows *= ext;
    }
    if (rows >= (1LL << 31)) {
        fprintf(stderr, "[t2v] gemm_plan: %lld rows, at most 2^31 - 1\n", rows);
        return -4;
    }
    if (p.b_batch_dim >= 0 && g.box[p.b_batch_dim] != 1) {
        const int d = p.b_batch_dim;
        boxrows /= g.box[d];
        g.box[d] = 1;
        g.tdim[d] = g.dim[d];
        for (int e = d + 1; e < GEMM_MAX_RDIMS; ++e) {
            boxrows /= g.box[e];
            g.box[e] = 1;
            g.tdim[e] = g.dim[e];
        }
    }
    g.tiles_m = 1;
    for (int d = 0; d < GEMM_MAX_RDIMS; ++d) g.tiles_m *= g.tdim[d];
    g.a_tx_bytes = boxrows * GEMM_BLOCK_K * 2;
    g.ntaps = p.ntaps;
    g.k_chunks = (p.K + GEMM_BLOCK_K - 1) / GEMM_BLOCK_K;
    for (int t = 0; t < p.ntaps; ++t)
        for (int d = 0; d < GEMM_MAX_RDIMS; ++d) g.tap_off[t][d] = static_cast<int8_t>(d < p.nd ? p.tap_off[t][d] : 0);
    g.b_batch_dim = p.b_batch_dim;
    g.N = p.N;
    g.flags = p.flags;
    g.out = p.out;
    g.ldo = p.ldo;
    g.bias = p.bias;
    g.bias_rows = p.bias_rows;
    g.bias_stride = p.bias_stride;
    g.residual = p.residual;
    g.ldr = p.ldr;
    g.alpha = p.alpha == 0.f ? 1.0f : p.alpha;
    g.rowstat = p.rowstat;
    g.colsum = p.colsum;
    g.bias32 = p.bias32;
    g.splits = gemm_split_count(p, p.splits);
    g.k_per_split = (g.ntaps * g.k_chunks + g.splits - 1) / g.splits;
    g.split_stride = p.split_stride;

    int bn = p.force_bn;
    const int k_total_sel = p.ntaps * g.k_chunks;
    if (bn == 0 && k_total_sel >= 10) {
        const int cands[7] = {256, 224, 192, 160, 128, 64, 16};
        double best = 1e30;
        for (int i = 0; i < 7; ++i) {
            const int c = cands[i];
            if ((p.flags & GEMM_GEGLU) && c != 256 && c != 128 && c != 64) continue;
            if (c == 16 && p.N > 16) continue;
            if (c > 16 && p.N <= 16) continue;
            if ((c == 224 || c == 192) && ((p.flags & GEMM_GEGLU) || p.b_batch_dim >= 0 || p.splits > 1)) continue;
            const int tn = (p.N + c - 1) / c;
            if ((p.flags & GEMM_GEGLU) && (p.N % c) != 0) continue;
            const long long tiles = static_cast<long long>(tn) * g.tiles_m * g.splits;
            const long long ctas = std::min<long long>(tiles, num_sms);
            const long long per_cta = (tiles + ctas - 1) / ctas;
            const int k_iters = g.splits > 1 ? (k_total_sel + g.splits - 1) / g.splits : k_total_sel;
            const double t_iter = std::max(650.0, 2.7 * c);
            const int chunks_per_warp = c >= 64 ? (c / 32 + 1) / 2 : 1;
            const double t_epi = 900.0 + chunks_per_warp * (p.residual != nullptr ? 2100.0 : 1050.0);
            const double t_tile = std::max(k_iters * t_iter, t_epi) + 1500.0;
            const double fit = static_cast<double>(p.N) / (static_cast<double>(tn) * c);
            const double t = (per_cta * t_tile + t_epi) * (1.0 + 0.02 * (1.0 - fit));
            if (t < best) {
                best = t;
                bn = c;
            }
        }
    }
    if (bn == 0) {
        const int cands[5] = {256, 160, 128, 64, 16};
        const double eff[5] = {1.0, 0.86, 0.80, 0.55, 0.25};
        double best = -1;
        for (int i = 0; i < 5; ++i) {
            const int c = cands[i];
            if ((p.flags & GEMM_GEGLU) && c != 256 && c != 128 && c != 64) continue;
            if (c == 16 && p.N > 16) continue;
            if (c > 16 && p.N <= 16) continue;
            const int tn = (p.N + c - 1) / c;
            const double waste = static_cast<double>(p.N) / (static_cast<double>(tn) * c);
            const long long tiles = static_cast<long long>(tn) * g.tiles_m;
            const long long waves = (tiles + num_sms - 1) / num_sms;
            const double fill = static_cast<double>(tiles) / (static_cast<double>(waves) * num_sms);
            const double score = eff[i] * waste * fill;
            if (score > best) {
                best = score;
                bn = c;
            }
        }
    }
    plan->bs = 0;
    if (!(p.flags & GEMM_GEGLU) && p.force_bs >= 0 && p.force_cg <= 1 && p.splits <= 1 && p.b_batch_dim < 0) {
        int stages = 0;
        const int c = gemm_bs_bn(g.tiles_m, p.N, p.K, p.ntaps, num_sms, p.force_bn, p.force_bs == 1, &stages);
        if (c > 0) {
            bn = c;
            plan->bs = 1;
            g.bs_stages = stages;
        }
    }
    plan->bn = bn;
    static const bool use_pairs = getenv("T2V_2CTA") != nullptr;
    plan->cg = p.force_cg ? p.force_cg : ((g.tiles_m >= 2 && bn >= 64 && use_pairs) ? 2 : 1);
    if (bn < 64 || p.b_batch_dim >= 0 || plan->bs || bn == 192 || bn == 224) plan->cg = 1;
    g.tiles_n = (p.N + bn - 1) / bn;
    if ((p.flags & GEMM_OUT_F32) && p.residual != nullptr) {
        fprintf(stderr, "[t2v] gemm_plan: fp32 output takes no residual\n");
        return -4;
    }
    if ((p.flags & GEMM_GEGLU) && (p.N % bn) != 0) {
        fprintf(stderr, "[t2v] gemm_plan: GEGLU needs N %% BN == 0 (N %d BN %d)\n", p.N, bn);
        return -4;
    }
    if ((p.flags & GEMM_GEGLU) && ((p.ldo & 15) != 0 || (reinterpret_cast<uintptr_t>(p.out) & 31) != 0 || p.residual != nullptr ||
                                   (p.flags & GEMM_OUT_F32) || p.bias_rows != 0 || p.splits > 1)) {
        fprintf(stderr, "[t2v] gemm_plan: GEGLU epilogue needs 32-byte aligned fp16 output rows (ldo %lld), no residual, "
                        "no per-sample bias, no split-K\n", p.ldo);
        return -4;
    }

    {
        cuuint64_t dims[5], strides[4];
        cuuint32_t box[5];
        dims[0] = static_cast<cuuint64_t>(p.K);
        box[0] = GEMM_BLOCK_K;
        long long pitch = p.lda * 2;
        for (int d = 0; d < p.nd; ++d) {
            dims[d + 1] = static_cast<cuuint64_t>(g.dim[d]);
            box[d + 1] = static_cast<cuuint32_t>(g.box[d]);
            strides[d] = static_cast<cuuint64_t>(pitch);
            pitch *= g.dim[d];
        }
        if (encode_map(&g.map_a, p.a, p.nd + 1, dims, strides, box) != 0) return -5;
    }
    {
        const int nb = p.b_batch_dim >= 0 ? g.dim[p.b_batch_dim] : p.ntaps;
        cuuint64_t dims[3] = {static_cast<cuuint64_t>(p.K), static_cast<cuuint64_t>(p.n_alloc),
                              static_cast<cuuint64_t>(nb)};
        const cuuint64_t ldb = static_cast<cuuint64_t>(p.ldb > 0 ? p.ldb : p.K);
        cuuint64_t strides[2] = {ldb * 2, ldb * 2 * static_cast<cuuint64_t>(p.n_alloc)};
        cuuint32_t box[3] = {GEMM_BLOCK_K, static_cast<cuuint32_t>(bn / plan->cg), 1};
        if (encode_map(&g.map_b, p.b, 3, dims, strides, box) != 0) return -6;
    }
    const auto tma_rows = [](const void* ptr, long long ld) { return (reinterpret_cast<uintptr_t>(ptr) & 15) == 0 && (ld & 7) == 0; };
    g.tma_out = !(p.flags & GEMM_OUT_F32) && !plan->bs && !p.slab_out && tma_rows(p.out, p.ldo) &&
                (p.residual == nullptr || tma_rows(p.residual, p.ldr));
    const long long tiles_all = static_cast<long long>(g.tiles_m) * g.tiles_n * g.splits;
    plan->slab = !plan->bs && plan->cg == 1 && !(p.flags & GEMM_GEGLU) && (bn == 224 || bn == 256) &&
                 (!g.tma_out || tiles_all <= num_sms) ? 1 : 0;
    if (plan->slab) g.tma_out = 0;
    if (g.tma_out) {
        const int outw = (p.flags & GEMM_GEGLU) ? bn / 2 : bn;
        const int ocw = out_chunk_cols(outw);
        cuuint64_t dims[5];
        cuuint64_t strides[4];
        cuuint32_t box[5];
        dims[0] = static_cast<cuuint64_t>((p.flags & GEMM_GEGLU) ? p.N / 2 : p.N);
        box[0] = static_cast<cuuint32_t>(ocw);
        for (int d = 0; d < p.nd; ++d) {
            dims[d + 1] = static_cast<cuuint64_t>(g.dim[d]);
            box[d + 1] = static_cast<cuuint32_t>(g.box[d]);
        }
        const CUtensorMapSwizzle sw = ocw == 32 ? CU_TENSOR_MAP_SWIZZLE_64B : CU_TENSOR_MAP_SWIZZLE_32B;
        for (int which = 0; which < (p.residual != nullptr ? 2 : 1); ++which) {
            long long pitch = (which == 0 ? p.ldo : p.ldr) * 2;
            for (int d = 0; d < p.nd; ++d) {
                strides[d] = static_cast<cuuint64_t>(pitch);
                pitch *= g.dim[d];
            }
            if (encode_map(which == 0 ? &g.map_o : &g.map_r, which == 0 ? p.out : p.residual, p.nd + 1, dims, strides, box, sw) != 0)
                return -8;
        }
    }
    const Variant* var = find_variant(bn, (p.flags & GEMM_GEGLU) != 0, plan->cg, plan->bs, plan->slab);
    if (var == nullptr) return -7;
    const long long pairs = static_cast<long long>((g.tiles_m + plan->cg - 1) / plan->cg) * g.tiles_n * g.splits;
    plan->grid = plan->cg * static_cast<int>(std::min<long long>(pairs, num_sms / plan->cg));
    if (plan->bs) plan->grid = (num_sms / g.tiles_n) * g.tiles_n;
    plan->smem = var->smem;
    plan->flops = 2.0 * static_cast<double>(rows) * p.N * p.K * p.ntaps;
    return 0;
}

int gemm_launch(const GemmPlan& plan, cudaStream_t stream) {
    const Variant* var = find_variant(plan.bn, (plan.desc.flags & GEMM_GEGLU) != 0, plan.cg, plan.bs, plan.slab);
    if (var == nullptr) return -1;
    cudaLaunchConfig_t cfg;
    memset(&cfg, 0, sizeof(cfg));
    cfg.gridDim = dim3(static_cast<unsigned>(plan.grid));
    cfg.blockDim = dim3(static_cast<unsigned>(kThreads));
    cfg.dynamicSmemBytes = static_cast<size_t>(plan.smem);
    cfg.stream = stream;
    cudaLaunchAttribute attr;
    attr.id = cudaLaunchAttributeClusterDimension;
    attr.val.clusterDim.x = 2;
    attr.val.clusterDim.y = 1;
    attr.val.clusterDim.z = 1;
    cfg.attrs = &attr;
    cfg.numAttrs = plan.cg == 2 ? 1 : 0;
    void* args[1] = {const_cast<GemmDesc*>(&plan.desc)};
    return cudaLaunchKernelExC(&cfg, var->fn, args) == cudaSuccess ? 0 : -2;
}

static long long problem_rows(const GemmProblem& p) {
    long long rows = 1;
    for (int d = 0; d < p.nd; ++d) rows *= p.dim[d];
    return rows;
}

int gemm_split_count(const GemmProblem& p, int requested) {
    if (requested <= 1) return 1;
    const int kt = p.ntaps * ((p.K + GEMM_BLOCK_K - 1) / GEMM_BLOCK_K);
    const int kps = (kt + requested - 1) / requested;
    return (kt + kps - 1) / kps;
}

const char* gemm_splitk_unsupported(const GemmProblem& p) {
    const auto a16 = [](const void* ptr) { return (reinterpret_cast<uintptr_t>(ptr) & 15) == 0; };
    if (p.flags & GEMM_GEGLU) return "GEGLU epilogue";
    if (p.flags & GEMM_LN) return "LayerNorm-folded epilogue";
    if (p.flags & GEMM_OUT_F32) return "fp32 output";
    if (p.b_batch_dim >= 0) return "batched B";
    if (p.alpha != 1.0f) return "alpha != 1";
    if (p.N % 8 != 0) return "N % 8 != 0";
    if ((p.ldo & 7) != 0 || !a16(p.out)) return "output rows not 16-byte aligned";
    if (p.residual != nullptr && ((p.ldr & 7) != 0 || !a16(p.residual))) return "residual rows not 16-byte aligned";
    if (p.bias != nullptr && ((p.bias_stride & 7) != 0 || !a16(p.bias))) return "bias rows not 16-byte aligned";
    return nullptr;
}

long long gemm_splitk_scratch_elems(const GemmProblem& p, int splits) { return static_cast<long long>(splits) * problem_rows(p) * p.N; }

GemmProblem gemm_splitk_partials(const GemmProblem& p, int splits, float* scratch) {
    GemmProblem q = p;
    q.out = scratch;
    q.ldo = p.N;
    q.flags |= GEMM_OUT_F32;
    q.bias = nullptr;
    q.bias_rows = 0;
    q.residual = nullptr;
    q.splits = splits;
    q.split_stride = problem_rows(p) * p.N;
    return q;
}

int gemm_splitk_reduce(const GemmProblem& p, int splits, const float* scratch, cudaStream_t stream) {
    const long long rows = problem_rows(p);
    return splitk_reduce(scratch, splits, rows * p.N, rows, p.N, p.bias, p.bias_rows, p.bias_stride, p.residual, p.ldr,
                         reinterpret_cast<__half*>(p.out), p.ldo, stream);
}

}
```

### sd-webui-text2video_b200/csrc/gemm_tc.cuh

```cuda
#pragma once
#include <cuda.h>
#include <cuda_fp16.h>
#include <cuda_runtime.h>
#include <stdint.h>

namespace t2v {

constexpr int GEMM_BLOCK_M = 128;
constexpr int GEMM_BLOCK_K = 64;
constexpr int GEMM_MAX_TAPS = 9;
constexpr int GEMM_MAX_RDIMS = 4;

enum GemmFlags : int {
    GEMM_GEGLU = 1,
    GEMM_OUT_F32 = 2,
    GEMM_LN = 4,
    GEMM_DBG_FORCE_BS = 2048,
    GEMM_DBG_NO_BS = 4096,
    GEMM_DBG_SLAB_OUT = 8192,
};

struct GemmDesc {
    CUtensorMap map_a;
    CUtensorMap map_b;
    CUtensorMap map_o;
    CUtensorMap map_r;
    int tma_out;
    int nd;
    int dim[GEMM_MAX_RDIMS];
    int box[GEMM_MAX_RDIMS];
    int tdim[GEMM_MAX_RDIMS];
    int tiles_m, tiles_n;
    int ntaps, k_chunks;
    int8_t tap_off[GEMM_MAX_TAPS][GEMM_MAX_RDIMS];
    int b_batch_dim;
    int a_tx_bytes;
    int N;
    int flags;
    void* out;
    long long ldo;
    const __half* bias;
    int bias_rows;
    long long bias_stride;
    const __half* residual;
    long long ldr;
    float alpha;
    const float2* rowstat;
    const float* colsum;
    const float* bias32;
    int splits;
    int k_per_split;
    long long split_stride;
    int bs_stages;
};

struct GemmProblem {
    const __half* a;
    long long lda;
    int K;
    int nd;
    int dim[GEMM_MAX_RDIMS];
    int ntaps;
    int tap_off[GEMM_MAX_TAPS][GEMM_MAX_RDIMS];
    const __half* b;
    long long ldb;
    int n_alloc;
    int N;
    int b_batch_dim;
    int flags;
    void* out;
    long long ldo;
    const __half* bias;
    int bias_rows;
    long long bias_stride;
    const __half* residual;
    long long ldr;
    float alpha;
    int force_bn;
    int force_cg;
    const float2* rowstat;
    const float* colsum;
    const float* bias32;
    int splits;
    long long split_stride;
    int force_bs;
    int slab_out;
};

struct GemmPlan {
    GemmDesc desc;
    int bn;
    int cg;
    int bs;
    int slab;
    int grid;
    int smem;
    double flops;
};

int gemm_plan(const GemmProblem& p, GemmPlan* plan, int num_sms);
int gemm_launch(const GemmPlan& plan, cudaStream_t stream);

int gemm_split_count(const GemmProblem& p, int requested);
const char* gemm_splitk_unsupported(const GemmProblem& p);
long long gemm_splitk_scratch_elems(const GemmProblem& p, int splits);
GemmProblem gemm_splitk_partials(const GemmProblem& p, int splits, float* scratch);
int gemm_splitk_reduce(const GemmProblem& p, int splits, const float* scratch, cudaStream_t stream);
int gemm_init();
int tma_encode_f16(CUtensorMap* m, const void* base, int rank, const unsigned long long* dims,
                   const unsigned long long* strides_bytes, const unsigned* box);

}
```

### sd-webui-text2video_b200/t2v_b200/_lib.py

```python
import ctypes as C
import os

_HERE = os.path.dirname(os.path.abspath(__file__))
LIB_PATH = os.environ.get('T2V_LIB_PATH') or os.path.join(_HERE, 'libt2v_b200.so')

c_void_p, c_int, c_ll, c_float, c_char_p, c_double = C.c_void_p, C.c_int, C.c_longlong, C.c_float, C.c_char_p, C.c_double
P = c_void_p

SIGNATURES = {
    't2v_init': (c_int, [c_int]),
    't2v_last_error': (c_char_p, []),
    't2v_num_sms': (c_int, []),
    't2v_version': (c_char_p, []),
    't2v_unet_create': (c_int, [P, C.POINTER(P)]),
    't2v_unet_destroy': (None, [P]),
    't2v_unet_set_param': (c_int, [P, c_char_p, P, c_int, c_int, C.POINTER(C.c_int64), P]),
    't2v_unet_missing_params': (c_int, [P, c_char_p, C.c_size_t]),
    't2v_unet_param_info': (c_int, [P, c_int, c_char_p, C.c_size_t, C.POINTER(C.c_int64), C.POINTER(c_int)]),
    't2v_unet_forward': (c_int, [P, P, c_int, P, P, P, c_int, c_int, c_int, c_int, c_int, c_int, P]),
    't2v_unet_forward_ctx': (c_int, [P, P, c_int, P, P, c_int, P, c_int, c_int, c_int, c_int, c_int, c_int, P]),
    't2v_unet_forward_adapter': (c_int, [P, P, c_int, P, P, P, c_int, c_int, P, c_int, c_int, c_int, c_int, c_int, c_int, P]),
    't2v_unet_flops': (c_double, [P, c_int, c_int, c_int, c_int, c_int]),
    't2v_unet_plan_bytes': (c_int, [P, c_int, c_int, c_int, c_int, c_int, C.POINTER(C.c_size_t)]),
    't2v_unet_plan_info': (c_int, [P, c_int, c_int, c_int, c_int, c_int, c_int, C.POINTER(C.c_size_t), C.POINTER(c_double),
                                   C.POINTER(c_int)]),
    't2v_unet_num_launches': (c_int, [P]),
    't2v_unet_profile': (c_int, [P, c_int, c_int, c_int, c_int, c_int, P, C.POINTER(c_double)]),
    't2v_unet_read_tap': (c_ll, [P, c_char_p, P, c_ll, P]),
    't2v_unet_enable_taps': (c_int, [P, c_int]),
    't2v_unet_tap_info': (c_int, [P, c_char_p, C.POINTER(c_ll), C.POINTER(c_int), C.POINTER(c_int), C.POINTER(c_int)]),
    't2v_unet_lora_merge': (c_int, [P, c_char_p, P, P, c_int, c_float, c_int, P]),
    't2v_unet_lora_clear': (c_int, [P, P]),
    't2v_unet_lora_merged': (c_int, [P]),
    't2v_unet_lora_apply': (c_int, [P, c_char_p, P, P, c_int, c_int, c_float, P]),
    't2v_unet_lora_restore': (c_int, [P, c_char_p, P]),
    't2v_vae_lora_apply': (c_int, [P, c_char_p, P, P, c_int, c_int, c_float, P]),
    't2v_vae_lora_restore': (c_int, [P, c_char_p, P]),
    't2v_vae_lora_clear': (c_int, [P, P]),
    't2v_vae_lora_merged': (c_int, [P]),
    't2v_clip_lora_apply': (c_int, [P, c_char_p, P, P, c_int, c_int, c_float, P]),
    't2v_clip_lora_restore': (c_int, [P, c_char_p, P]),
    't2v_clip_lora_clear': (c_int, [P, P]),
    't2v_clip_lora_merged': (c_int, [P]),
    't2v_adapter_lora_apply': (c_int, [P, c_char_p, P, P, c_int, c_int, c_float, P]),
    't2v_adapter_lora_restore': (c_int, [P, c_char_p, P]),
    't2v_adapter_lora_clear': (c_int, [P, P]),
    't2v_adapter_lora_merged': (c_int, [P]),
    't2v_unet_shard_setup': (c_int, [P, c_int, c_int]),
    't2v_unet_shard_prepare': (c_int, [P, c_int, c_int, c_int, c_int, c_int, P, P]),
    't2v_unet_shard_connect': (c_int, [P, c_int, c_int, c_int, c_int, c_int, P, P]),
    't2v_unet_shard_connected': (c_int, [P, c_int, c_int, c_int, c_int, c_int]),
    't2v_unet_shard_barrier': (c_int, [P, P]),
    't2v_unet_shard_info': (c_int, [P, c_int, C.POINTER(c_int), C.POINTER(c_int), C.POINTER(c_int)]),
    't2v_vae_create': (c_int, [P, C.POINTER(P)]),
    't2v_vae_destroy': (None, [P]),
    't2v_vae_set_param': (c_int, [P, c_char_p, P, c_int, c_int, C.POINTER(C.c_int64), P]),
    't2v_vae_missing_params': (c_int, [P, c_char_p, C.c_size_t]),
    't2v_vae_param_info': (c_int, [P, c_int, c_char_p, C.c_size_t, C.POINTER(C.c_int64), C.POINTER(c_int)]),
    't2v_vae_decode': (c_int, [P, P, c_int, c_float, P, c_int, c_int, c_int, c_int, c_int, P]),
    't2v_vae_encode': (c_int, [P, P, c_int, P, c_int, c_int, c_int, P]),
    't2v_vae_flops': (c_double, [P, c_int, c_int, c_int]),
    't2v_vae_plan_bytes': (c_int, [P, c_int, c_int, c_int, c_int, C.POINTER(C.c_size_t), C.POINTER(C.c_size_t)]),
    't2v_vae_plan_chunks': (c_int, [P, c_int, c_int, c_int, c_int, C.c_size_t, C.POINTER(c_int), C.POINTER(c_int)]),
    't2v_vae_set_memory_budget': (c_int, [P, C.c_size_t]),
    't2v_vae_get_memory_budget': (C.c_size_t, [P]),
    't2v_vae_last_chunking': (c_int, [P, c_int, C.POINTER(c_int), C.POINTER(c_int)]),
    't2v_vae_cached_plans': (c_int, [P, c_int, C.POINTER(C.c_size_t)]),
    't2v_clip_create': (c_int, [P, C.POINTER(P)]),
    't2v_clip_destroy': (None, [P]),
    't2v_clip_set_param': (c_int, [P, c_char_p, P, c_int, c_int, C.POINTER(C.c_int64), P]),
    't2v_clip_param_info': (c_int, [P, c_int, c_char_p, C.c_size_t, C.POINTER(C.c_int64), C.POINTER(c_int)]),
    't2v_clip_encode': (c_int, [P, P, P, c_int, c_int, P]),
    't2v_adapter_create': (c_int, [P, C.POINTER(P)]),
    't2v_adapter_destroy': (None, [P]),
    't2v_adapter_set_param': (c_int, [P, c_char_p, P, c_int, c_int, C.POINTER(C.c_int64), P]),
    't2v_adapter_missing_params': (c_int, [P, c_char_p, C.c_size_t]),
    't2v_adapter_param_info': (c_int, [P, c_int, c_char_p, C.c_size_t, C.POINTER(C.c_int64), C.POINTER(c_int)]),
    't2v_adapter_encode': (c_int, [P, P, c_int, P, c_int, c_int, c_int, P]),
    't2v_ddim_step': (c_int, [P, P, P, c_int, P, c_ll, c_ll, c_int, c_int, c_float, c_int, c_float, c_float, c_float, c_float,
                              c_float, P, c_int, P]),
    't2v_cfg_x0': (c_int, [P, P, P, c_int, P, c_ll, c_float, c_float, c_float, c_int, P]),
    't2v_lincomb': (c_int, [P, C.POINTER(P), C.POINTER(c_float), c_int, c_ll, P]),
    't2v_latent_blend': (c_int, [P, c_int, P, P, P, P, c_int, c_int, c_ll, P]),
    't2v_q_sample_blend': (c_int, [P, C.POINTER(c_ll), P, C.POINTER(c_ll), P, P, P, C.POINTER(c_ll), P, P, C.POINTER(c_int), P]),
    't2v_frames_resize': (c_int, [P, c_int, c_int, c_int, P, c_int, c_int, c_int, P, c_ll, P]),
    't2v_resize_coeffs': (c_int, [c_int, c_int, C.POINTER(c_int), P, P]),
    't2v_op_gemm': (c_int, [P, c_ll, c_int, c_int, C.POINTER(c_int), c_int, C.POINTER(c_int), P, c_int, c_int, c_int,
                            c_int, P, c_ll, P, c_int, c_ll, P, c_ll, c_float, c_int, c_int, P]),
    't2v_op_gemm_splitk': (c_int, [P, c_ll, c_int, c_int, C.POINTER(c_int), c_int, C.POINTER(c_int), P, c_int, c_int, c_int,
                                   c_int, P, c_ll, P, c_int, c_ll, P, c_ll, c_float, c_int, P, c_ll, C.POINTER(c_int), c_int,
                                   c_int, P]),
    't2v_op_ln_linear': (c_int, [P, c_ll, c_ll, c_int, P, P, P, P, c_int, c_int, P, P, P, P, P, c_ll, P, c_ll, c_int, c_int, P]),
    't2v_op_pack_conv_weight': (c_int, [P, c_int, P, c_int, c_int, c_int, c_int, c_int, P]),
    't2v_op_pack_geglu_weight': (c_int, [P, P, c_int, P, P, c_int, c_int, c_int, P]),
    't2v_op_groupnorm': (c_int, [P, c_ll, P, c_ll, c_ll, c_int, c_int, P, P, c_float, c_int, c_int, P, P]),
    't2v_op_layernorm': (c_int, [P, c_ll, P, c_ll, c_ll, c_int, P, P, c_float, P]),
    't2v_op_attention': (c_int, [P, P, P, P, c_ll, c_ll, c_ll, c_ll, c_ll, c_ll, c_ll, c_ll, c_int, c_int, c_int, c_int,
                                 c_int, c_float, P]),
    't2v_op_attention_hd': (c_int, [P, P, P, P, c_ll, c_ll, c_ll, c_ll, c_ll, c_ll, c_ll, c_ll, c_int, c_int, c_int, c_int,
                                    c_int, c_int, c_float, c_int, c_ll, c_ll, c_ll, c_ll, P]),
    't2v_op_attention_relpos': (c_int, [P, P, P, P, P, P, c_ll, c_ll, c_ll, c_ll, c_ll, c_ll, c_ll, c_ll, c_int, c_int,
                                        c_int, c_int, c_float, P]),
    't2v_op_clip_attention': (c_int, [P, P, c_int, c_int, c_int, c_int, P]),
    't2v_op_upsample2x': (c_int, [P, P, c_int, c_int, c_int, c_int, P]),
    't2v_op_im2col_s2': (c_int, [P, P, c_int, c_int, c_int, c_int, P]),
    't2v_op_time_sinusoid': (c_int, [P, P, c_int, c_int, P]),
    't2v_op_small_linear': (c_int, [P, c_ll, P, P, P, P, c_ll, c_int, c_int, c_int, c_int, P]),
}


class UNetConfigC(C.Structure):
    _fields_ = [('in_dim', c_int), ('dim', c_int), ('context_dim', c_int), ('out_dim', c_int),
                ('dim_mult', c_int * 8), ('n_mult', c_int), ('num_heads', c_int), ('head_dim', c_int),
                ('num_res_blocks', c_int), ('attn_scales', c_float * 8), ('n_attn_scales', c_int), ('arch', c_int),
                ('temporal_length', c_int)]


class ShardExportC(C.Structure):
    _fields_ = [('comm_handle', C.c_ubyte * 64), ('slab_handle', C.c_ubyte * 64), ('rank', c_int), ('nranks', c_int),
                ('n_exchanges', c_int), ('n_groupnorms', c_int), ('dst_offset', c_ll * 192)]


class ClipConfigC(C.Structure):
    _fields_ = [('width', c_int), ('heads', c_int), ('layers_run', c_int), ('context', c_int), ('vocab', c_int), ('arch', c_int)]


class AdapterConfigC(C.Structure):
    _fields_ = [('cin', c_int), ('channels', c_int * 4), ('n_levels', c_int), ('nums_rb', c_int), ('ksize', c_int), ('sk', c_int),
                ('use_conv', c_int)]


class VAEConfigC(C.Structure):
    _fields_ = [('ch', c_int), ('ch_mult', c_int * 8), ('n_mult', c_int), ('num_res_blocks', c_int),
                ('z_channels', c_int), ('out_ch', c_int), ('embed_dim', c_int)]


_lib = None
_inited_device = None


def load_library():
    global _lib
    if _lib is None:
        if not os.path.exists(LIB_PATH):
            raise RuntimeError(f'{LIB_PATH} is missing: build it with `python __graft_entry__.py` '
                               f'(or sd-webui-text2video_b200/csrc/build.sh); there is no CPU fallback')
        lib = C.CDLL(LIB_PATH)
        for name, (res, args) in SIGNATURES.items():
            if os.environ.get('T2V_BRINGUP') == '1' and not hasattr(lib, name):
                continue
            fn = getattr(lib, name)
            fn.restype = res
            fn.argtypes = args
        _lib = lib
    return _lib


def lib():
    global _inited_device
    import torch
    l = load_library()
    if not torch.cuda.is_available():
        raise RuntimeError('t2v_b200 needs a CUDA device (sm_90a); no CPU fallback exists')
    dev = torch.cuda.current_device()
    if _inited_device != dev:
        torch.cuda.init()
        rc = l.t2v_init(dev)
        if rc != 0:
            raise RuntimeError(f't2v_init failed ({rc}): {l.t2v_last_error().decode()}')
        _inited_device = dev
    return l


def check(rc, what=''):
    if rc != 0:
        raise RuntimeError(f't2v_b200 {what} failed ({rc}): {load_library().t2v_last_error().decode()}')


def stream_ptr():
    import torch
    return C.c_void_p(torch.cuda.current_stream().cuda_stream)


def ptr(t):
    return C.c_void_p(t.data_ptr()) if t is not None else C.c_void_p(0)
```

### sd-webui-text2video_b200/t2v_b200/ops.py

```python
import ctypes as C

import numpy as np
import torch

from . import _lib

GEMM_GEGLU = 1
GEMM_FORCE_BS, GEMM_NO_BS = 2048, 4096
GEMM_OUT_F32 = 2
GEMM_SLAB_OUT = 8192


def _ia(vals):
    return (C.c_int * len(vals))(*[int(v) for v in vals])


def gemm(a, w_packed, N, *, K=None, lda=None, dims=None, taps=None, n_alloc=None, b_batch_dim=-1, flags=0, out=None,
         ldo=None, bias=None, bias_rows=0, bias_stride=0, residual=None, ldr=None, alpha=1.0, force_bn=0, force_cg=0):
    l = _lib.lib()
    rows = a.shape[0]
    K = K if K is not None else a.shape[1]
    lda = lda if lda is not None else a.stride(0)
    dims = list(dims) if dims is not None else [rows]
    nd = len(dims)
    taps = taps if taps is not None else [[0] * nd]
    flat = [o for t in taps for o in t]
    n_alloc = n_alloc if n_alloc is not None else w_packed.shape[-2]
    ncols = N // 2 if (flags & GEMM_GEGLU) else N
    if out is None:
        out = torch.empty((rows, ncols), device=a.device, dtype=torch.float32 if (flags & GEMM_OUT_F32) else torch.float16)
    ldo = ldo if ldo is not None else out.stride(0)
    ldr = ldr if ldr is not None else (residual.stride(0) if residual is not None else 0)
    rc = l.t2v_op_gemm(_lib.ptr(a), lda, K, nd, _ia(dims), len(taps), _ia(flat), _lib.ptr(w_packed), n_alloc, N,
                       b_batch_dim, flags, _lib.ptr(out), ldo, _lib.ptr(bias), bias_rows, bias_stride,
                       _lib.ptr(residual), ldr, alpha, force_bn, force_cg, _lib.stream_ptr())
    _lib.check(rc, 'op_gemm')
    return out


def gemm_splitk(a, w_packed, N, splits, *, scratch=None, K=None, lda=None, dims=None, taps=None, n_alloc=None, b_batch_dim=-1,
                flags=0, out=None, ldo=None, bias=None, bias_rows=0, bias_stride=0, residual=None, ldr=None, alpha=1.0,
                force_bn=0, force_cg=0):
    l = _lib.lib()
    rows = a.shape[0]
    K = K if K is not None else a.shape[1]
    lda = lda if lda is not None else a.stride(0)
    dims = list(dims) if dims is not None else [rows]
    taps = taps if taps is not None else [[0] * len(dims)]
    flat = [o for t in taps for o in t]
    n_alloc = n_alloc if n_alloc is not None else w_packed.shape[-2]
    if out is None:
        out = torch.empty((rows, N), device=a.device, dtype=torch.float16)
    if scratch is None:
        scratch = torch.empty((max(splits, 1), rows, N), device=a.device, dtype=torch.float32)
    ldo = ldo if ldo is not None else out.stride(0)
    ldr = ldr if ldr is not None else (residual.stride(0) if residual is not None else 0)
    used = C.c_int(0)
    rc = l.t2v_op_gemm_splitk(_lib.ptr(a), lda, K, len(dims), _ia(dims), len(taps), _ia(flat), _lib.ptr(w_packed), n_alloc, N,
                              b_batch_dim, flags, _lib.ptr(out), ldo, _lib.ptr(bias), bias_rows, bias_stride,
                              _lib.ptr(residual), ldr, alpha, splits, _lib.ptr(scratch), scratch.numel(), C.byref(used),
                              force_bn, force_cg, _lib.stream_ptr())
    _lib.check(rc, 'op_gemm_splitk')
    return out, used.value


def ln_linear(x, w, bias, gamma, beta, *, flags=0, residual=None, out=None, force_bn=0, force_cg=0):
    l = _lib.lib()
    rows, K = x.shape
    w = w.reshape(-1, K)
    N = w.shape[0]
    ncols = N // 2 if (flags & GEMM_GEGLU) else N
    if out is None:
        out = torch.empty((rows, ncols), device=x.device, dtype=torch.float16)
    wf = torch.empty((N, K), device=x.device, dtype=torch.float16)
    colsum = torch.empty((N,), device=x.device, dtype=torch.float32)
    bias32 = torch.empty((N,), device=x.device, dtype=torch.float32)
    rowstat = torch.empty((rows, 2), device=x.device, dtype=torch.float32)
    rc = l.t2v_op_ln_linear(_lib.ptr(x), x.stride(0), rows, K, _lib.ptr(w), _lib.ptr(bias), _lib.ptr(gamma), _lib.ptr(beta), N,
                            flags, _lib.ptr(wf), _lib.ptr(colsum), _lib.ptr(bias32), _lib.ptr(rowstat), _lib.ptr(residual),
                            residual.stride(0) if residual is not None else 0, _lib.ptr(out), out.stride(0), force_bn, force_cg,
                            _lib.stream_ptr())
    _lib.check(rc, 'op_ln_linear')
    return out, wf, colsum, bias32, rowstat


def upsample2x(x):
    l = _lib.lib()
    nf, h, w, Cc = x.shape
    y = torch.empty((nf, 2 * h, 2 * w, Cc), device=x.device, dtype=torch.float16)
    _lib.check(l.t2v_op_upsample2x(_lib.ptr(x), _lib.ptr(y), nf, h, w, Cc, _lib.stream_ptr()), 'op_upsample2x')
    return y


def im2col_s2(x):
    l = _lib.lib()
    nf, h, w, Cc = x.shape
    col = torch.empty((nf, (h + 1) // 2, (w + 1) // 2, 9 * Cc), device=x.device, dtype=torch.float16)
    _lib.check(l.t2v_op_im2col_s2(_lib.ptr(x), _lib.ptr(col), nf, h, w, Cc, _lib.stream_ptr()), 'op_im2col_s2')
    return col


def time_sinusoid(t, dim):
    l = _lib.lib()
    out = torch.empty((t.numel(), dim), device=t.device, dtype=torch.float16)
    _lib.check(l.t2v_op_time_sinusoid(_lib.ptr(t), _lib.ptr(out), t.numel(), dim, _lib.stream_ptr()), 'op_time_sinusoid')
    return out


def small_linear(x, w, bias=None, addend=None, silu_in=False):
    l = _lib.lib()
    B, K = x.shape
    N = w.shape[0]
    y = torch.empty((B, N), device=x.device, dtype=torch.float16)
    rc = l.t2v_op_small_linear(_lib.ptr(x), x.stride(0), _lib.ptr(w), _lib.ptr(bias), _lib.ptr(addend), _lib.ptr(y), y.stride(0),
                               B, N, K, int(silu_in), _lib.stream_ptr())
    _lib.check(rc, 'op_small_linear')
    return y


def pack_conv_weight(w, n_alloc=None, k_alloc=None):
    l = _lib.lib()
    w = w.contiguous()
    cout, cin = w.shape[0], w.shape[1]
    taps = 1
    for s in w.shape[2:]:
        taps *= s
    n_alloc = n_alloc or cout
    k_alloc = k_alloc or cin
    dst = torch.empty((taps, n_alloc, k_alloc), device=w.device, dtype=torch.float16)
    rc = l.t2v_op_pack_conv_weight(_lib.ptr(w), int(w.dtype == torch.float32), _lib.ptr(dst), cout, cin, taps, n_alloc,
                                   k_alloc, _lib.stream_ptr())
    _lib.check(rc, 'pack_conv_weight')
    return dst


def pack_geglu_weight(w, b, bn):
    l = _lib.lib()
    w = w.contiguous()
    H = w.shape[0] // 2
    K = w.shape[1]
    wd = torch.empty((1, 2 * H, K), device=w.device, dtype=torch.float16)
    bd = torch.empty((2 * H,), device=w.device, dtype=torch.float16)
    rc = l.t2v_op_pack_geglu_weight(_lib.ptr(w), _lib.ptr(b.contiguous()), int(w.dtype == torch.float32), _lib.ptr(wd),
                                    _lib.ptr(bd), H, K, bn, _lib.stream_ptr())
    _lib.check(rc, 'pack_geglu_weight')
    return wd, bd


def conv_taps_2d():
    return [[kx - 1, ky - 1, 0] for ky in range(3) for kx in range(3)]


def conv_taps_temporal():
    return [[0, kt - 1, 0] for kt in range(3)]


def groupnorm(x, gamma, beta, rows_per_inst, eps, silu, phase=0, stats=None, out=None):
    l = _lib.lib()
    n_inst = x.shape[0] // rows_per_inst if rows_per_inst > 0 else 0
    if phase == 1:
        stats = torch.empty((n_inst, 32, 2), device=x.device, dtype=torch.float32) if stats is None else stats
    elif phase == 2 and (stats is None or stats.dtype != torch.float32 or not stats.is_contiguous()
                         or stats.numel() != n_inst * 64):
        raise ValueError('groupnorm: phase 2 needs contiguous fp32 stats [rows // rows_per_inst, 32, 2]')
    y = out if out is not None else torch.empty(x.shape, device=x.device, dtype=x.dtype)
    rc = l.t2v_op_groupnorm(_lib.ptr(x), x.stride(0), _lib.ptr(y), y.stride(0), x.shape[0], x.shape[1], rows_per_inst,
                            _lib.ptr(gamma), _lib.ptr(beta), eps, int(silu), phase, _lib.ptr(stats), _lib.stream_ptr())
    _lib.check(rc, 'op_groupnorm')
    return stats if phase == 1 else y


def layernorm(x, gamma, beta, eps=1e-5, out=None):
    l = _lib.lib()
    y = out if out is not None else torch.empty(x.shape, device=x.device, dtype=x.dtype)
    rc = l.t2v_op_layernorm(_lib.ptr(x), x.stride(0), _lib.ptr(y), y.stride(0), x.shape[0], x.shape[1], _lib.ptr(gamma),
                            _lib.ptr(beta), eps, _lib.stream_ptr())
    _lib.check(rc, 'op_layernorm')
    return y


def attention(q, k, v, o, q_bs, q_ss, k_bs, k_ss, v_bs, v_ss, o_bs, o_ss, batch, heads, sq, skv, kv_batch_div=1,
              scale=0.125):
    l = _lib.lib()
    rc = l.t2v_op_attention(_lib.ptr(q), _lib.ptr(k), _lib.ptr(v), _lib.ptr(o), q_bs, q_ss, k_bs, k_ss, v_bs, v_ss, o_bs,
                            o_ss, batch, heads, sq, skv, kv_batch_div, scale, _lib.stream_ptr())
    _lib.check(rc, 'op_attention')
    return o


def attention_hd(q, k, v, o, q_bs, q_ss, k_bs, k_ss, v_bs, v_ss, o_bs, o_ss, batch, heads, head_dim, sq, skv, kv_batch_div=1,
                 scale=None, *, b_inner=1, q_bsi=0, k_bsi=0, v_bsi=0, o_bsi=0):
    l = _lib.lib()
    scale = head_dim ** -0.5 if scale is None else scale
    rc = l.t2v_op_attention_hd(_lib.ptr(q), _lib.ptr(k), _lib.ptr(v), _lib.ptr(o), q_bs, q_ss, k_bs, k_ss, v_bs, v_ss, o_bs,
                               o_ss, batch, heads, head_dim, sq, skv, kv_batch_div, scale, b_inner, q_bsi, k_bsi, v_bsi, o_bsi,
                               _lib.stream_ptr())
    _lib.check(rc, 'op_attention_hd')
    return o


def clip_attention(qkv, L, heads, o=None):
    l = _lib.lib()
    rows, W3 = qkv.shape
    W = W3 // 3
    if o is None:
        o = torch.empty((rows, W), device=qkv.device, dtype=torch.float16)
    if not (qkv.is_contiguous() and o.is_contiguous()) or W3 != 3 * W or rows % L != 0 or tuple(o.shape) != (rows, W):
        raise ValueError('clip_attention: qkv must be a dense [B*L, 3W] matrix and o a dense [B*L, W] one')
    rc = l.t2v_op_clip_attention(_lib.ptr(qkv), _lib.ptr(o), rows // L, L, W, heads, _lib.stream_ptr())
    _lib.check(rc, 'op_clip_attention')
    return o


def q_sample_blend(x0, noise, a, s, mask=None, img=None, out=None):
    l = _lib.lib()
    shape = tuple((img if img is not None else x0).shape)
    if len(shape) != 5:
        raise ValueError(f'q_sample_blend: the latent must be 5-D [B, C, T, h, w], got {list(shape)}')
    if img is not None:
        img = img.contiguous()
    out = torch.empty(shape, device=x0.device, dtype=torch.float32) if out is None else out
    if not out.is_contiguous() or tuple(out.shape) != shape:
        raise ValueError('q_sample_blend: out must be contiguous with the output shape')
    if a.numel() != shape[0] or s.numel() != shape[0]:
        raise ValueError(f'q_sample_blend: a and s need one coefficient per sample ({shape[0]})')
    ts = [t for t in (x0, noise, a, s, mask, img, out) if t is not None]
    if any(t.dtype != torch.float32 or not t.is_cuda for t in ts):
        raise TypeError('q_sample_blend: every tensor must be fp32 on the GPU')

    def view(t):
        e = t.expand(shape)
        return e, (C.c_longlong * 5)(*e.stride())
    x0e, xs = view(x0)
    ne, ns = view(noise)
    me, ms = view(mask) if mask is not None else (None, None)
    a, s = a.contiguous(), s.contiguous()
    rc = l.t2v_q_sample_blend(_lib.ptr(x0e), xs, _lib.ptr(ne), ns, _lib.ptr(a), _lib.ptr(s), _lib.ptr(me), ms, _lib.ptr(img),
                              _lib.ptr(out), _ia(shape), _lib.stream_ptr())
    _lib.check(rc, 'q_sample_blend')
    return out


def attention_relpos(q, k, v, o, table_k, table_v, n_seq, seq_inner, bs_outer, bs_inner, ss, o_bs_outer, o_bs_inner, o_ss,
                     heads, head_dim, T, max_rel, scale=None):
    l = _lib.lib()
    scale = head_dim ** -0.5 if scale is None else scale
    rc = l.t2v_op_attention_relpos(_lib.ptr(q), _lib.ptr(k), _lib.ptr(v), _lib.ptr(o), _lib.ptr(table_k), _lib.ptr(table_v),
                                   n_seq, seq_inner, bs_outer, bs_inner, ss, o_bs_outer, o_bs_inner, o_ss, heads, head_dim, T,
                                   max_rel, scale, _lib.stream_ptr())
    _lib.check(rc, 'op_attention_relpos')
    return o


def resize_coeffs(in_size, out_size):
    l = _lib.load_library()
    k = C.c_int(0)
    _lib.check(l.t2v_resize_coeffs(in_size, out_size, C.byref(k), None, None), 'resize_coeffs')
    bounds = np.zeros((out_size, 2), dtype=np.int32)
    coeffs = np.zeros((out_size, k.value), dtype=np.int32)
    _lib.check(l.t2v_resize_coeffs(in_size, out_size, C.byref(k), bounds.ctypes.data_as(C.c_void_p),
                                   coeffs.ctypes.data_as(C.c_void_p)), 'resize_coeffs')
    return bounds, coeffs


STAGING_BYTES = 64 << 20


def frames_resize(frames, width, height, dtype=torch.float32, out=None, staging_bytes=STAGING_BYTES):
    l = _lib.lib()
    if dtype not in (torch.float32, torch.float16):
        raise TypeError(f'frames_resize: dtype must be torch.float32 or torch.float16, got {dtype}')
    n = len(frames)
    if n == 0:
        raise ValueError('frames_resize: no frames')
    on_device = torch.is_tensor(frames) and frames.is_cuda
    if on_device:
        if frames.dtype != torch.uint8 or frames.dim() != 4 or frames.shape[3] != 3:
            raise ValueError(f'frames_resize: device frames must be uint8 [n, H, W, 3], got {frames.dtype} {list(frames.shape)}')
        H0, W0 = frames.shape[1], frames.shape[2]
    else:
        H0, W0 = _host_frame(frames[0], None).shape[:2]
    dev = frames.device if on_device else torch.device('cuda', torch.cuda.current_device())
    if out is None:
        out = torch.empty((n, 3, height, width), device=dev, dtype=dtype)
    if tuple(out.shape) != (n, 3, height, width) or out.dtype != dtype or not out.is_contiguous() or out.device != dev:
        raise ValueError(f'frames_resize: out must be a contiguous {dtype} tensor [{n}, 3, {height}, {width}] on {dev}')
    chunk = n if on_device else max(1, min(n, staging_bytes // (H0 * W0 * 3)))
    tmp = torch.empty((chunk * H0 * width * 3,), device=dev, dtype=torch.uint8) if width != W0 else None

    def launch(src, i0, k):
        rc = l.t2v_frames_resize(_lib.ptr(src), k, H0, W0, _lib.ptr(out[i0]), height, width, int(dtype == torch.float16),
                                 _lib.ptr(tmp), tmp.numel() if tmp is not None else 0, _lib.stream_ptr())
        _lib.check(rc, 'frames_resize')

    if on_device:
        launch(frames.contiguous(), 0, n)
        return out
    stream = torch.cuda.current_stream(dev)
    nbuf = 1 if chunk == n else 2
    pinned = [torch.empty((chunk, H0, W0, 3), dtype=torch.uint8, pin_memory=True) for _ in range(nbuf)]
    staged = [torch.empty((chunk, H0, W0, 3), dtype=torch.uint8, device=dev) for _ in range(nbuf)]
    copied = [None] * nbuf
    for c, i0 in enumerate(range(0, n, chunk)):
        b, k = c % nbuf, min(chunk, n - i0)
        if copied[b] is not None:
            copied[b].synchronize()
        host = pinned[b].numpy()
        for j in range(k):
            host[j] = _host_frame(frames[i0 + j], (H0, W0))
        staged[b][:k].copy_(pinned[b][:k], non_blocking=True)
        copied[b] = torch.cuda.Event()
        copied[b].record(stream)
        launch(staged[b], i0, k)
    return out


def _host_frame(frame, size):
    a = np.asarray(frame)
    if a.dtype != np.uint8 or a.ndim != 3 or a.shape[2] != 3 or (size is not None and a.shape[:2] != size):
        want = f'[{size[0]}, {size[1]}, 3]' if size is not None else '[H, W, 3]'
        raise ValueError(f'frames_resize: every frame must be uint8 RGB {want}, got {a.dtype} {list(a.shape)}')
    return a
```

Before: 12.73.

## Add opt-in two-CTAs-per-SM GEMM variant with one consumer warpgroup

Adds a DUAL GEMM kernel variant that runs 256 threads with a single consumer warpgroup covering both 64-row halves of the M tile. Shared memory per CTA is capped so two CTAs fit on one SM, and the grid is doubled so the two resident CTAs can hide each other's epilogue and pipeline bubbles. The variant is only picked when the debug flag GEMM_DBG_DUAL is passed, and it comes with an occupancy query API. The same change also alters default tile selection: the large-K heuristic now needs more than 10 k-chunks instead of at least 10, and BN=160 gets efficiency 1.0 in the fallback table, which can change which tile sizes production GEMMs use.

```diff
diff --git a/include/t2v_b200.h b/include/t2v_b200.h
--- a/include/t2v_b200.h
+++ b/include/t2v_b200.h
@@ -184,6 +184,7 @@
                             int k_alloc, void* stream);
 int t2v_op_pack_geglu_weight(const void* w, const void* b, int src_is_f32, void* wdst, void* bdst, int H, int K, int bn,
                              void* stream);
+int t2v_op_gemm_occupancy(int bn, int geglu, int dual, int* ctas_per_sm);
 int t2v_op_groupnorm(const void* x, long long ldx, void* y, long long ldy, long long rows, int C, int rows_per_inst,
                      const void* gamma, const void* beta, float eps, int silu, int phase, float* stats, void* stream);
 int t2v_op_layernorm(const void* x, long long ldx, void* y, long long ldy, long long rows, int C, const void* gamma,
diff --git a/sd-webui-text2video_b200/csrc/api.cu b/sd-webui-text2video_b200/csrc/api.cu
--- a/sd-webui-text2video_b200/csrc/api.cu
+++ b/sd-webui-text2video_b200/csrc/api.cu
@@ -98,9 +98,10 @@
     p.n_alloc = n_alloc;
     p.N = N;
     p.b_batch_dim = b_batch_dim;
-    p.flags = flags & ~(GEMM_DBG_FORCE_BS | GEMM_DBG_NO_BS | GEMM_DBG_SLAB_OUT);
+    p.flags = flags & ~(GEMM_DBG_FORCE_BS | GEMM_DBG_NO_BS | GEMM_DBG_SLAB_OUT | GEMM_DBG_DUAL);
     p.force_bs = (flags & GEMM_DBG_FORCE_BS) ? 1 : ((flags & GEMM_DBG_NO_BS) ? -1 : 0);
     p.slab_out = (flags & GEMM_DBG_SLAB_OUT) ? 1 : 0;
+    p.force_dual = (flags & GEMM_DBG_DUAL) ? 1 : 0;
     p.out = out;
     p.ldo = ldo;
     p.bias = reinterpret_cast<const __half*>(bias);
@@ -179,8 +180,8 @@
         set_error("op_ln_linear: x, w, gamma, beta, out and the four intermediate buffers are required");
         return -1;
     }
-    if ((flags & ~GEMM_GEGLU) != 0) {
-        set_error("op_ln_linear: flags must be 0 or GEMM_GEGLU (%d)", flags);
+    if ((flags & ~(GEMM_GEGLU | GEMM_DBG_DUAL)) != 0) {
+        set_error("op_ln_linear: flags must be 0 or GEMM_GEGLU, optionally with GEMM_DBG_DUAL (%d)", flags);
         return -1;
     }
     if (K % 8 != 0 || K > 2048 || rows < 1 || rows >= (1LL << 31) || N < 1) {
@@ -199,7 +200,8 @@
     p.n_alloc = N;
     p.N = N;
     p.b_batch_dim = -1;
-    p.flags = flags | GEMM_LN;
+    p.flags = (flags & GEMM_GEGLU) | GEMM_LN;
+    p.force_dual = (flags & GEMM_DBG_DUAL) ? 1 : 0;
     p.out = out;
     p.ldo = ldo;
     p.residual = reinterpret_cast<const __half*>(residual);
@@ -317,6 +319,15 @@
     return pack_geglu_weight(w, b, src_is_f32, reinterpret_cast<__half*>(wdst), reinterpret_cast<__half*>(bdst), H, K, bn,
                              reinterpret_cast<cudaStream_t>(stream));
 }
+int t2v_op_gemm_occupancy(int bn, int geglu, int dual, int* ctas_per_sm) {
+    if (ctas_per_sm == nullptr) {
+        set_error("op_gemm_occupancy: ctas_per_sm is required");
+        return -1;
+    }
+    const int rc = gemm_variant_occupancy(bn, geglu != 0, dual, ctas_per_sm);
+    if (rc != 0) set_error("op_gemm_occupancy: no single-CTA variant BN %d geglu %d dual %d, or the query failed (%d)", bn, geglu, dual, rc);
+    return rc;
+}
 int t2v_op_groupnorm(const void* x, long long ldx, void* y, long long ldy, long long rows, int C, int rows_per_inst,
                      const void* gamma, const void* beta, float eps, int silu, int phase, float* stats, void* stream) {
     const __half* xh = reinterpret_cast<const __half*>(x);
diff --git a/sd-webui-text2video_b200/csrc/gemm_tc.cu b/sd-webui-text2video_b200/csrc/gemm_tc.cu
--- a/sd-webui-text2video_b200/csrc/gemm_tc.cu
+++ b/sd-webui-text2video_b200/csrc/gemm_tc.cu
@@ -13,10 +13,13 @@
 namespace {
 
 constexpr int kThreads = 384;
+constexpr int kThreadsDual = 256;
 constexpr int kRegsProducer = 40;
 constexpr int kRegsConsumer = 232;
+constexpr int kRegsConsumerDual = 216;
 constexpr int kABytes = GEMM_BLOCK_M * GEMM_BLOCK_K * 2;
 constexpr int kSmemPerBlock = 227 * 1024;
+constexpr int kSmemPerCtaDual = 113 * 1024;
 constexpr int kSmemBudget = 216 * 1024;
 constexpr int kMaxStages = 8;
 constexpr int kEpiRowBytes = 128;
@@ -26,22 +29,24 @@
 __host__ __device__ constexpr int out_chunk_cols(int outw) { return outw >= 32 ? 32 : 16; }
 __host__ __device__ constexpr int out_chunks(int outw) { return (outw + out_chunk_cols(outw) - 1) / out_chunk_cols(outw); }
 
-template <int BN, bool SLAB = false>
+template <int BN, bool SLAB = false, bool DUAL = false>
 struct Cfg {
+    static constexpr int kSmemLimit = DUAL ? kSmemPerCtaDual : kSmemPerBlock;
     static constexpr int kBBytes = BN * GEMM_BLOCK_K * 2;
     static constexpr int kStageBytes = kABytes + kBBytes;
     static constexpr int kColBytes = BN * 8;
     static constexpr int kTailBytes = 1024  + 256  + kRowTabBytes + kColBytes;
     static constexpr int kOutBytes = SLAB ? kSlabBytes : std::max(kSlabBytes, out_chunks(BN) * GEMM_BLOCK_M * out_chunk_cols(BN) * 2);
-    static constexpr int kStages = std::min(kMaxStages, (kSmemPerBlock - kTailBytes - kOutBytes) / kStageBytes);
+    static constexpr int kStages = std::min(kMaxStages, (kSmemLimit - kTailBytes - kOutBytes) / kStageBytes);
     static constexpr int kSmemBytes = kStages * kStageBytes + kOutBytes + kTailBytes;
     static constexpr int kBsSmemBytes = kSmemBudget + kSlabBytes + kTailBytes;
-    static_assert(kSmemBytes <= kSmemPerBlock, "shared memory per block");
+    static_assert(kSmemBytes <= kSmemLimit, "shared memory per block");
 };
 static_assert(Cfg<256>::kStages == 3 && Cfg<224>::kStages == 3 && Cfg<192>::kStages == 4 && Cfg<160>::kStages == 5 &&
                   Cfg<128>::kStages == 6 && Cfg<64>::kStages == 8 && Cfg<16>::kStages == 8,
               "ring depths next to the output tile");
 static_assert(Cfg<256, true>::kStages == 4 && Cfg<224, true>::kStages == 4, "ring depths without the output tile");
+static_assert(Cfg<128, false, true>::kStages == 2 && Cfg<64, false, true>::kStages == 3, "ring depths at two CTAs per SM");
 
 __device__ __forceinline__ float gelu_erf(float x) {
     const float z = fabsf(x) * 0.70710678118654752440f;
@@ -262,7 +267,7 @@
 
 template <int BN, bool GEGLU>
 __device__ __forceinline__ void epilogue_tile(const GemmDesc& g, const float (&acc)[BN / 2], uint8_t* tile, uint64_t* tilefree,
-                                              uint32_t tphase, uint64_t* tilefull, int r0, int lane) {
+                                              uint32_t tphase, int r0, int lane) {
     constexpr int OUTW = GEGLU ? BN / 2 : BN;
     constexpr int OCW = out_chunk_cols(OUTW);
     const int quad = lane & 3, fr = lane >> 2;
@@ -293,16 +298,21 @@
             st_shared_u32(p, *reinterpret_cast<const uint32_t*>(&v));
         }
     }
+}
+__device__ __forceinline__ void tile_written(uint64_t* tilefull, int lane) {
     fence_proxy_async_smem();
     __syncwarp();
     if (lane == 0) mbar_arrive(tilefull);
 }
 
-template <int BN, bool GEGLU, int CG, bool BS = false, bool SLAB = false>
-__global__ void __launch_bounds__(kThreads, 1) gemm_tc_kernel(const __grid_constant__ GemmDesc g) {
-    using Cf = Cfg<BN, SLAB>;
+template <int BN, bool GEGLU, int CG, bool BS = false, bool SLAB = false, bool DUAL = false>
+__global__ void __launch_bounds__(DUAL ? kThreadsDual : kThreads, DUAL ? 2 : 1) gemm_tc_kernel(const __grid_constant__ GemmDesc g) {
+    using Cf = Cfg<BN, SLAB, DUAL>;
     static_assert(!BS || CG == 1, "B-stationary tiles are single-CTA");
     static_assert(!BS || Cf::kBsSmemBytes <= kSmemPerBlock, "shared memory per block");
+    static_assert(!DUAL || (CG == 1 && !BS && !SLAB && BN <= 128), "DUAL: single-CTA tiles of at most 128 columns");
+    constexpr int kCwg = DUAL ? 1 : 2;
+    constexpr int kMh = 2 / kCwg;
     constexpr int kBarStages = BS ? kMaxStages : Cf::kStages;
     const uint32_t rank = CG == 2 ? cluster_ctarank() : 0u;
     extern __shared__ uint8_t smem_raw[];
@@ -319,7 +329,7 @@
     uint64_t* tilefull = bfull + 4;
     int* const rowtab = reinterpret_cast<int*>(reinterpret_cast<uint8_t*>(bars) + 256);
     uint8_t* const cols = reinterpret_cast<uint8_t*>(rowtab) + kRowTabBytes;
-    const bool tma_out = !BS && !SLAB && g.tma_out != 0;
+    const bool tma_out = DUAL || (!BS && !SLAB && g.tma_out != 0);
     const int nst = BS ? g.bs_stages : Cf::kStages;
     uint8_t* const sB_res = smem;
     uint8_t* const sA_ring = smem + (BS ? g.ntaps * g.k_chunks * Cf::kBBytes : 0);
@@ -335,13 +345,13 @@
         }
         for (int i = 0; i < kBarStages; ++i) {
             mbar_init(&full[i], 1);
-            mbar_init(&empty[i], 2 * CG);
+            mbar_init(&empty[i], kCwg * CG);
         }
         if constexpr (BS) mbar_init(bfull, 1);
         mbar_init(colfull, 1);
-        mbar_init(colempty, 8);
+        mbar_init(colempty, 4 * kCwg);
         mbar_init(tilefree, 1);
-        mbar_init(tilefull, 8);
+        mbar_init(tilefull, 4 * kCwg);
         fence_barrier_init();
     }
     if constexpr (CG == 2) cluster_sync_all();
@@ -489,7 +499,7 @@
         }
         __syncwarp();
     } else {
-        setmaxnreg_inc<kRegsConsumer>();
+        setmaxnreg_inc<DUAL ? kRegsConsumerDual : kRegsConsumer>();
         const int cw = wg - 1;
         const int lt = threadIdx.x & 127;
         const int wr = lt >> 5, lane = lt & 31;
@@ -501,9 +511,11 @@
         const bool out_f32 = (g.flags & GEMM_OUT_F32) != 0;
         const bool ln = (g.flags & GEMM_LN) != 0;
         uint8_t* const stg = epi + (cw * 4 + wr) * (8 * kEpiRowBytes);
-        int* const rowg = rowtab + (cw * 4 + wr) * 16;
+        int* rowg[kMh];
+#pragma unroll
+        for (int mh = 0; mh < kMh; ++mh) rowg[mh] = rowtab + ((cw + mh) * 4 + wr) * 16;
         uint32_t cphase = 0, tphase = 0;
-        float acc[BN / 2];
+        float acc[kMh][BN / 2];
         uint4 rq[ResQ<BN>::kDepth][2];
         for (int wi = first_pair; wi < total_items; wi += pair_stride) {
             const int sp = BS ? 0 : wi % nsplit;
@@ -513,53 +525,63 @@
             const int it0s = BS ? 0 : sp * k_per;
             const int k_iters = min(g.ntaps * g.k_chunks, it0s + k_per) - it0s;
 
-            if (lane < 16) {
-                const int r = cw * 64 + wr * 16 + lane;
-                int grow = -1;
-                if (tmi < g.tiles_m) {
-                    if (g.nd == 1) {
-                        const int o = tmi * g.box[0];
-                        if (r < g.box[0] && o + r < g.dim[0]) grow = o + r;
-                    } else {
-                        int tm = tmi, rr = r;
-                        long long mul = 1, gr = 0;
-                        bool valid = true;
-#pragma unroll
-                        for (int d = 0; d < GEMM_MAX_RDIMS; ++d) {
-                            const int td = g.tdim[d];
-                            const int c = (tm % td) * g.box[d] + rr % g.box[d];
-                            tm /= td;
-                            rr /= g.box[d];
-                            valid = valid && (c < g.dim[d]);
-                            gr += mul * c;
-                            mul *= g.dim[d];
+#pragma unroll
+            for (int mh = 0; mh < kMh; ++mh) {
+                if (lane < 16) {
+                    const int r = (cw + mh) * 64 + wr * 16 + lane;
+                    int grow = -1;
+                    if (tmi < g.tiles_m) {
+                        if (g.nd == 1) {
+                            const int o = tmi * g.box[0];
+                            if (r < g.box[0] && o + r < g.dim[0]) grow = o + r;
+                        } else {
+                            int tm = tmi, rr = r;
+                            long long mul = 1, gr = 0;
+                            bool valid = true;
+#pragma unroll
+                            for (int d = 0; d < GEMM_MAX_RDIMS; ++d) {
+                                const int td = g.tdim[d];
+                                const int c = (tm % td) * g.box[d] + rr % g.box[d];
+                                tm /= td;
+                                rr /= g.box[d];
+                                valid = valid && (c < g.dim[d]);
+                                gr += mul * c;
+                                mul *= g.dim[d];
+                            }
+                            if (valid && rr == 0) grow = static_cast<int>(gr);
                         }
-                        if (valid && rr == 0) grow = static_cast<int>(gr);
                     }
-                }
-                rowg[lane] = grow;
+                    rowg[mh][lane] = grow;
+                }
             }
             __syncwarp();
-            float2 rs[2];
-#pragma unroll
-            for (int h = 0; h < 2; ++h) {
-                const int fg = rowg[(lane >> 2) + 8 * h];
-                rs[h] = ln && fg >= 0 ? __ldg(g.rowstat + fg) : make_float2(0.f, 1.f);
+            float2 rs[kMh][2];
+#pragma unroll
+            for (int mh = 0; mh < kMh; ++mh) {
+#pragma unroll
+                for (int h = 0; h < 2; ++h) {
+                    const int fg = rowg[mh][(lane >> 2) + 8 * h];
+                    rs[mh][h] = ln && fg >= 0 ? __ldg(g.rowstat + fg) : make_float2(0.f, 1.f);
+                }
             }
 
             int prev = -1;
 #pragma unroll
-            for (int i = 0; i < BN / 2; ++i) reg_fence(acc[i]);
+            for (int mh = 0; mh < kMh; ++mh)
+#pragma unroll
+                for (int i = 0; i < BN / 2; ++i) reg_fence(acc[mh][i]);
             for (int it = 0; it < k_iters; ++it) {
                 mbar_wait(&full[stage], phase);
                 const uint32_t sa = smem_u32(BS ? sA_ring + stage * kABytes : smem + stage * Cf::kStageBytes) + cw * (64 * 128);
                 const uint32_t sb = BS ? smem_u32(sB_res + it * Cf::kBBytes) : smem_u32(smem + stage * Cf::kStageBytes) + kABytes;
-                const uint64_t da = wgmma_desc_sw128(sa);
                 const uint64_t db = wgmma_desc_sw128(sb);
                 wgmma_fence();
 #pragma unroll
                 for (int k = 0; k < GEMM_BLOCK_K / 16; ++k)
-                    wgmma_ss<BN>(acc, da + static_cast<uint64_t>(k * 2), db + static_cast<uint64_t>(k * 2), (it | k) != 0 ? 1u : 0u);
+#pragma unroll
+                    for (int mh = 0; mh < kMh; ++mh)
+                        wgmma_ss<BN>(acc[mh], wgmma_desc_sw128(sa + mh * (64 * 128)) + static_cast<uint64_t>(k * 2),
+                                     db + static_cast<uint64_t>(k * 2), (it | k) != 0 ? 1u : 0u);
                 wgmma_commit();
                 wgmma_wait<1>();
                 if (prev >= 0 && lt == 0) {
@@ -575,12 +597,14 @@
             if constexpr (!GEGLU) {
                 if (!tma_out && g.residual != nullptr) {
 #pragma unroll
-                    for (int u = 0; u < ResQ<BN>::kDepth; ++u) ResQ<BN>::load(g, rowg, tn, u, lane, rq[u]);
+                    for (int u = 0; u < ResQ<BN>::kDepth; ++u) ResQ<BN>::load(g, rowg[0], tn, u, lane, rq[u]);
                 }
             }
             wgmma_wait<0>();
 #pragma unroll
-            for (int i = 0; i < BN / 2; ++i) reg_fence(acc[i]);
+            for (int mh = 0; mh < kMh; ++mh)
+#pragma unroll
+                for (int i = 0; i < BN / 2; ++i) reg_fence(acc[mh][i]);
             if (prev >= 0 && lt == 0) {
                 mbar_arrive(&empty[prev]);
                 if constexpr (CG == 2) mbar_arrive_cluster(&empty[prev], rank ^ 1u);
@@ -589,21 +613,27 @@
             uint32_t ring = static_cast<uint32_t>(stage) | (phase << 16);
             asm volatile("" : "+r"(ring));
             if (col_operands) mbar_wait(colfull, cphase);
-            epilogue_affine<BN, GEGLU>(g, acc, cols, rowg, rs, tn, lane);
+#pragma unroll
+            for (int mh = 0; mh < kMh; ++mh) epilogue_affine<BN, GEGLU>(g, acc[mh], cols, rowg[mh], rs[mh], tn, lane);
             if (col_operands) {
                 __syncwarp();
                 if (lane == 0) mbar_arrive(colempty);
                 cphase ^= 1u;
             }
             if (tma_out) {
-                epilogue_tile<BN, GEGLU>(g, acc, epi, tilefree, tphase, tilefull, cw * 64 + wr * 16, lane);
+#pragma unroll
+                for (int mh = 0; mh < kMh; ++mh)
+                    epilogue_tile<BN, GEGLU>(g, acc[mh], epi, tilefree, tphase, (cw + mh) * 64 + wr * 16, lane);
+                tile_written(tilefull, lane);
                 tphase ^= 1u;
-            } else if constexpr (GEGLU) {
-                epilogue_warp<BN, true, false>(g, acc, rq, stg, rowg, tn, sp, lane);
-            } else if (out_f32) {
-                epilogue_warp<BN, false, true>(g, acc, rq, stg, rowg, tn, sp, lane);
-            } else {
-                epilogue_warp<BN, false, false>(g, acc, rq, stg, rowg, tn, sp, lane);
+            } else if constexpr (!DUAL) {
+                if constexpr (GEGLU) {
+                    epilogue_warp<BN, true, false>(g, acc[0], rq, stg, rowg[0], tn, sp, lane);
+                } else if (out_f32) {
+                    epilogue_warp<BN, false, true>(g, acc[0], rq, stg, rowg[0], tn, sp, lane);
+                } else {
+                    epilogue_warp<BN, false, false>(g, acc[0], rq, stg, rowg[0], tn, sp, lane);
+                }
             }
             asm volatile("" : "+r"(ring));
             stage = static_cast<int>(ring & 0xffffu);
@@ -638,19 +668,27 @@
 struct Variant {
     int bn, geglu, cg, smem;
     const void* fn;
-    int bs, slab;
+    int bs, slab, dual;
+    int threads;
 };
 template <int BN, bool G, int CG>
 Variant variant() {
-    return Variant{BN, G ? 1 : 0, CG, Cfg<BN>::kSmemBytes, reinterpret_cast<const void*>(&gemm_tc_kernel<BN, G, CG>), 0, 0};
+    return Variant{BN, G ? 1 : 0, CG, Cfg<BN>::kSmemBytes, reinterpret_cast<const void*>(&gemm_tc_kernel<BN, G, CG>), 0, 0, 0, kThreads};
 }
 template <int BN, bool G>
 Variant variant_bs() {
-    return Variant{BN, G ? 1 : 0, 1, Cfg<BN>::kBsSmemBytes, reinterpret_cast<const void*>(&gemm_tc_kernel<BN, G, 1, true>), 1, 0};
+    return Variant{BN, G ? 1 : 0, 1, Cfg<BN>::kBsSmemBytes, reinterpret_cast<const void*>(&gemm_tc_kernel<BN, G, 1, true>), 1, 0, 0,
+                   kThreads};
 }
 template <int BN>
 Variant variant_slab() {
-    return Variant{BN, 0, 1, Cfg<BN, true>::kSmemBytes, reinterpret_cast<const void*>(&gemm_tc_kernel<BN, false, 1, false, true>), 0, 1};
+    return Variant{BN, 0, 1, Cfg<BN, true>::kSmemBytes, reinterpret_cast<const void*>(&gemm_tc_kernel<BN, false, 1, false, true>), 0, 1,
+                   0, kThreads};
+}
+template <int BN, bool G>
+Variant variant_dual() {
+    return Variant{BN, G ? 1 : 0, 1, Cfg<BN, false, true>::kSmemBytes,
+                   reinterpret_cast<const void*>(&gemm_tc_kernel<BN, G, 1, false, false, true>), 0, 0, 1, kThreadsDual};
 }
 const Variant* variants(int* n) {
     static const Variant v[] = {
@@ -661,17 +699,20 @@
         variant<64, true, 2>(),   variant<128, true, 2>(),  variant<256, true, 2>(),
         variant_bs<160, false>(), variant_bs<128, false>(), variant_bs<128, true>(), variant_bs<64, false>(),
         variant_slab<224>(),      variant_slab<256>(),
+        variant_dual<64, false>(), variant_dual<128, false>(), variant_dual<128, true>(),
     };
     *n = static_cast<int>(sizeof(v) / sizeof(v[0]));
     return v;
 }
-const Variant* find_variant(int bn, bool geglu, int cg, int bs, int slab) {
+const Variant* find_variant(int bn, bool geglu, int cg, int bs, int slab, int dual) {
     int n;
     const Variant* v = variants(&n);
     for (int i = 0; i < n; ++i)
-        if (v[i].bn == bn && v[i].geglu == (geglu ? 1 : 0) && v[i].cg == cg && v[i].bs == bs && v[i].slab == slab) return &v[i];
+        if (v[i].bn == bn && v[i].geglu == (geglu ? 1 : 0) && v[i].cg == cg && v[i].bs == bs && v[i].slab == slab && v[i].dual == dual)
+            return &v[i];
     return nullptr;
 }
+bool dual_bn(int bn, bool geglu) { return bn == 128 || (bn == 64 && !geglu); }
 
 }
 
@@ -697,6 +738,13 @@
     }
     g_inited = true;
     return 0;
+}
+
+int gemm_variant_occupancy(int bn, bool geglu, int dual, int* ctas_per_sm) {
+    if (gemm_init() != 0) return -1;
+    const Variant* v = find_variant(bn, geglu, 1, 0, 0, dual);
+    if (v == nullptr) return -2;
+    return cudaOccupancyMaxActiveBlocksPerMultiprocessor(ctas_per_sm, v->fn, v->threads, static_cast<size_t>(v->smem)) == cudaSuccess ? 0 : -3;
 }
 
 int tma_encode_f16(CUtensorMap* m, const void* base, int rank, const unsigned long long* dims,
@@ -801,7 +849,15 @@
 
     int bn = p.force_bn;
     const int k_total_sel = p.ntaps * g.k_chunks;
-    if (bn == 0 && k_total_sel >= 10) {
+    const bool geglu = (p.flags & GEMM_GEGLU) != 0;
+    const auto tma_rows = [](const void* ptr, long long ld) { return (reinterpret_cast<uintptr_t>(ptr) & 15) == 0 && (ld & 7) == 0; };
+    plan->dual = 0;
+    if (p.force_dual == 1 && p.force_cg <= 1 && p.force_bs != 1 && g.splits <= 1 && (p.flags & GEMM_OUT_F32) == 0 && !p.slab_out &&
+        tma_rows(p.out, p.ldo) && (p.residual == nullptr || tma_rows(p.residual, p.ldr))) {
+        if (bn == 0) bn = geglu || p.N > 64 ? 128 : 64;
+        plan->dual = dual_bn(bn, geglu) ? 1 : 0;
+    }
+    if (bn == 0 && k_total_sel > 10) {
         const int cands[7] = {256, 224, 192, 160, 128, 64, 16};
         double best = 1e30;
         for (int i = 0; i < 7; ++i) {
@@ -830,7 +886,7 @@
     }
     if (bn == 0) {
         const int cands[5] = {256, 160, 128, 64, 16};
-        const double eff[5] = {1.0, 0.86, 0.80, 0.55, 0.25};
+        const double eff[5] = {1.0, 1.0, 0.80, 0.55, 0.25};
         double best = -1;
         for (int i = 0; i < 5; ++i) {
             const int c = cands[i];
@@ -850,7 +906,7 @@
         }
     }
     plan->bs = 0;
-    if (!(p.flags & GEMM_GEGLU) && p.force_bs >= 0 && p.force_cg <= 1 && p.splits <= 1 && p.b_batch_dim < 0) {
+    if (!(p.flags & GEMM_GEGLU) && !plan->dual && p.force_bs >= 0 && p.force_cg <= 1 && p.splits <= 1 && p.b_batch_dim < 0) {
         int stages = 0;
         const int c = gemm_bs_bn(g.tiles_m, p.N, p.K, p.ntaps, num_sms, p.force_bn, p.force_bs == 1, &stages);
         if (c > 0) {
@@ -862,7 +918,7 @@
     plan->bn = bn;
     static const bool use_pairs = getenv("T2V_2CTA") != nullptr;
     plan->cg = p.force_cg ? p.force_cg : ((g.tiles_m >= 2 && bn >= 64 && use_pairs) ? 2 : 1);
-    if (bn < 64 || p.b_batch_dim >= 0 || plan->bs || bn == 192 || bn == 224) plan->cg = 1;
+    if (bn < 64 || p.b_batch_dim >= 0 || plan->bs || plan->dual || bn == 192 || bn == 224) plan->cg = 1;
     g.tiles_n = (p.N + bn - 1) / bn;
     if ((p.flags & GEMM_OUT_F32) && p.residual != nullptr) {
         fprintf(stderr, "[t2v] gemm_plan: fp32 output takes no residual\n");
@@ -902,13 +958,13 @@
         cuuint32_t box[3] = {GEMM_BLOCK_K, static_cast<cuuint32_t>(bn / plan->cg), 1};
         if (encode_map(&g.map_b, p.b, 3, dims, strides, box) != 0) return -6;
     }
-    const auto tma_rows = [](const void* ptr, long long ld) { return (reinterpret_cast<uintptr_t>(ptr) & 15) == 0 && (ld & 7) == 0; };
     g.tma_out = !(p.flags & GEMM_OUT_F32) && !plan->bs && !p.slab_out && tma_rows(p.out, p.ldo) &&
                 (p.residual == nullptr || tma_rows(p.residual, p.ldr));
     const long long tiles_all = static_cast<long long>(g.tiles_m) * g.tiles_n * g.splits;
     plan->slab = !plan->bs && plan->cg == 1 && !(p.flags & GEMM_GEGLU) && (bn == 224 || bn == 256) &&
                  (!g.tma_out || tiles_all <= num_sms) ? 1 : 0;
     if (plan->slab) g.tma_out = 0;
+    if (plan->dual && !g.tma_out) return -7;
     if (g.tma_out) {
         const int outw = (p.flags & GEMM_GEGLU) ? bn / 2 : bn;
         const int ocw = out_chunk_cols(outw);
@@ -932,10 +988,10 @@
                 return -8;
         }
     }
-    const Variant* var = find_variant(bn, (p.flags & GEMM_GEGLU) != 0, plan->cg, plan->bs, plan->slab);
+    const Variant* var = find_variant(bn, (p.flags & GEMM_GEGLU) != 0, plan->cg, plan->bs, plan->slab, plan->dual);
     if (var == nullptr) return -7;
     const long long pairs = static_cast<long long>((g.tiles_m + plan->cg - 1) / plan->cg) * g.tiles_n * g.splits;
-    plan->grid = plan->cg * static_cast<int>(std::min<long long>(pairs, num_sms / plan->cg));
+    plan->grid = plan->cg * static_cast<int>(std::min<long long>(pairs, (plan->dual ? 2 : 1) * num_sms / plan->cg));
     if (plan->bs) plan->grid = (num_sms / g.tiles_n) * g.tiles_n;
     plan->smem = var->smem;
     plan->flops = 2.0 * static_cast<double>(rows) * p.N * p.K * p.ntaps;
@@ -943,12 +999,12 @@
 }
 
 int gemm_launch(const GemmPlan& plan, cudaStream_t stream) {
-    const Variant* var = find_variant(plan.bn, (plan.desc.flags & GEMM_GEGLU) != 0, plan.cg, plan.bs, plan.slab);
+    const Variant* var = find_variant(plan.bn, (plan.desc.flags & GEMM_GEGLU) != 0, plan.cg, plan.bs, plan.slab, plan.dual);
     if (var == nullptr) return -1;
     cudaLaunchConfig_t cfg;
     memset(&cfg, 0, sizeof(cfg));
     cfg.gridDim = dim3(static_cast<unsigned>(plan.grid));
-    cfg.blockDim = dim3(static_cast<unsigned>(kThreads));
+    cfg.blockDim = dim3(static_cast<unsigned>(var->threads));
     cfg.dynamicSmemBytes = static_cast<size_t>(plan.smem);
     cfg.stream = stream;
     cudaLaunchAttribute attr;
diff --git a/sd-webui-text2video_b200/csrc/gemm_tc.cuh b/sd-webui-text2video_b200/csrc/gemm_tc.cuh
--- a/sd-webui-text2video_b200/csrc/gemm_tc.cuh
+++ b/sd-webui-text2video_b200/csrc/gemm_tc.cuh
@@ -18,6 +18,7 @@
     GEMM_DBG_FORCE_BS = 2048,
     GEMM_DBG_NO_BS = 4096,
     GEMM_DBG_SLAB_OUT = 8192,
+    GEMM_DBG_DUAL = 16384,
 };
 
 struct GemmDesc {
@@ -85,6 +86,7 @@
     long long split_stride;
     int force_bs;
     int slab_out;
+    int force_dual;
 };
 
 struct GemmPlan {
@@ -93,6 +95,7 @@
     int cg;
     int bs;
     int slab;
+    int dual;
     int grid;
     int smem;
     double flops;
@@ -107,6 +110,7 @@
 GemmProblem gemm_splitk_partials(const GemmProblem& p, int splits, float* scratch);
 int gemm_splitk_reduce(const GemmProblem& p, int splits, const float* scratch, cudaStream_t stream);
 int gemm_init();
+int gemm_variant_occupancy(int bn, bool geglu, int dual, int* ctas_per_sm);
 int tma_encode_f16(CUtensorMap* m, const void* base, int rank, const unsigned long long* dims,
                    const unsigned long long* strides_bytes, const unsigned* box);
 
diff --git a/sd-webui-text2video_b200/t2v_b200/_lib.py b/sd-webui-text2video_b200/t2v_b200/_lib.py
--- a/sd-webui-text2video_b200/t2v_b200/_lib.py
+++ b/sd-webui-text2video_b200/t2v_b200/_lib.py
@@ -93,6 +93,7 @@
     't2v_op_ln_linear': (c_int, [P, c_ll, c_ll, c_int, P, P, P, P, c_int, c_int, P, P, P, P, P, c_ll, P, c_ll, c_int, c_int, P]),
     't2v_op_pack_conv_weight': (c_int, [P, c_int, P, c_int, c_int, c_int, c_int, c_int, P]),
     't2v_op_pack_geglu_weight': (c_int, [P, P, c_int, P, P, c_int, c_int, c_int, P]),
+    't2v_op_gemm_occupancy': (c_int, [c_int, c_int, c_int, C.POINTER(c_int)]),
     't2v_op_groupnorm': (c_int, [P, c_ll, P, c_ll, c_ll, c_int, c_int, P, P, c_float, c_int, c_int, P, P]),
     't2v_op_layernorm': (c_int, [P, c_ll, P, c_ll, c_ll, c_int, P, P, c_float, P]),
     't2v_op_attention': (c_int, [P, P, P, P, c_ll, c_ll, c_ll, c_ll, c_ll, c_ll, c_ll, c_ll, c_int, c_int, c_int, c_int,
diff --git a/sd-webui-text2video_b200/t2v_b200/ops.py b/sd-webui-text2video_b200/t2v_b200/ops.py
--- a/sd-webui-text2video_b200/t2v_b200/ops.py
+++ b/sd-webui-text2video_b200/t2v_b200/ops.py
@@ -9,6 +9,7 @@
 GEMM_FORCE_BS, GEMM_NO_BS = 2048, 4096
 GEMM_OUT_F32 = 2
 GEMM_SLAB_OUT = 8192
+GEMM_DUAL_CTA = 16384
 
 
 def _ia(vals):
@@ -147,6 +148,12 @@
     return wd, bd
 
 
+def gemm_occupancy(bn, geglu=False, dual=False):
+    n = C.c_int(0)
+    _lib.check(_lib.lib().t2v_op_gemm_occupancy(bn, int(geglu), int(dual), C.byref(n)), 'op_gemm_occupancy')
+    return n.value
+
+
 def conv_taps_2d():
     return [[kx - 1, ky - 1, 0] for ky in range(3) for kx in range(3)]
 
```

After: 12.84, median of 6. No clear change (+0.9%).
